# cselab/odil

Measured on AMD Instinct MI355X. Metric: grid-point-updates/s, Poisson 512^3 multigrid, higher is better.
Workload: dtype f64

## Files before the change

### include/odil_hip.h

```cpp
#ifndef ODIL_HIP_H
#define ODIL_HIP_H

#include <stddef.h>
#include <stdint.h>

#ifdef __cplusplus
extern "C" {
#endif

#define ODIL_MAX_NDIM 4
#define ODIL_MAX_LEVELS 32
#define ODIL_E_INVAL (-1)
#define ODIL_E_LAUNCH (-2)
#define ODIL_E_NODEV (-3)

const char* odil_last_error(void);
int odil_version(void);
int odil_device_count(void);
size_t odil_reduce_workspace_bytes(void);

int odil_interp_add_f64(const double* coarse, const double* add, double* fine, const int64_t* cshape, int ndim,
                        const char* loc, double coarse_scale, double add_scale, void* stream);
int odil_interp_add_f32(const float* coarse, const float* add, float* fine, const int64_t* cshape, int ndim,
                        const char* loc, float coarse_scale, float add_scale, void* stream);
// ... 116 lines not shown
size_t odil_poisson_residual_synth_workspace_bytes(const int64_t* cshape);
int odil_poisson_residual_synth_f64(const double* coarse, const double* w0, const double* rhs, double* fu,
                                    const int64_t* cshape, const double* h2, int64_t z0, int64_t z1, double denom,
                                    double* partials, double* column_sums, size_t column_sums_size, double* loss,
                                    void* stream);
int odil_poisson_residual_synth_f32(const float* coarse, const float* w0, const float* rhs, float* fu,
                                    const int64_t* cshape, const float* h2, int64_t z0, int64_t z1, double denom,
                                    double* partials, double* column_sums, size_t column_sums_size, float* loss,
                                    void* stream);

int odil_poisson_jacobi_synth_f64(const double* coarse, const double* x, const double* rhs, double* xout,
                                  const int64_t* cshape, const double* h2, double omega, void* stream);
int odil_poisson_jacobi_synth_f32(const float* coarse, const float* x, const float* rhs, float* xout,
                                  const int64_t* cshape, const float* h2, float omega, void* stream);

int odil_poisson_adjoint_f64(const double* fu, double* gu, const int64_t* shape, int ndim, const double* h2,
                             double scale, void* stream);
int odil_poisson_adjoint_f32(const float* fu, float* gu, const int64_t* shape, int ndim, const float* h2,
                             float scale, void* stream);
int odil_poisson_adjoint_adam_f64(const double* fu, double* gu, double* x, double* m, double* v, const int64_t* shape,
                                  int ndim, const double* h2, double scale, double alpha, double one_minus_b1,
                                  double one_minus_b2, double eps, const double* alpha_dev, void* stream);
int odil_poisson_adjoint_adam_f32(const float* fu, float* gu, float* x, float* m, float* v, const int64_t* shape,
                                  int ndim, const float* h2, float scale, float alpha, float one_minus_b1,
                                  float one_minus_b2, float eps, const float* alpha_dev, void* stream);
int odil_poisson_jac_coeffs_f64(double* coeffs, const int64_t* shape, int ndim, const double* h2, void* stream);
int odil_poisson_jac_coeffs_f32(float* coeffs, const int64_t* shape, int ndim, const float* h2, void* stream);
int odil_poisson_jac_match_f64(const double* const* arrays, const int64_t* shape, int ndim, const double* h2,
                               double* partials, double* out, void* stream);
int odil_poisson_jac_match_f32(const float* const* arrays, const int64_t* shape, int ndim, const float* h2, double* partials,
                               float* out, void* stream);

int odil_adam_step_f64(double* x, double* m, double* v, const double* g, int64_t n, double alpha,
                       double one_minus_b1, double one_minus_b2, double eps, const double* alpha_dev, void* stream);
int odil_adam_step_f32(float* x, float* m, float* v, const float* g, int64_t n, float alpha, float one_minus_b1,
                       float one_minus_b2, float eps, const float* alpha_dev, void* stream);
int odil_adam_step_pieces_f64(double* x, double* m, double* v, const double* g, int64_t npieces, int64_t stride,
                              int64_t offset, int64_t count, double alpha, double one_minus_b1, double one_minus_b2,
                              double eps, const double* alpha_dev, void* stream);
int odil_adam_step_pieces_f32(float* x, float* m, float* v, const float* g, int64_t npieces, int64_t stride,
                              int64_t offset, int64_t count, float alpha, float one_minus_b1, float one_minus_b2,
                              float eps, const float* alpha_dev, void* stream);
int odil_planes_copy_f64(double* arr, double* buf, const int64_t* descs, int ndesc, int64_t max_count, int vec_ok,
                         int mode, void* stream);
int odil_planes_copy_f32(float* arr, float* buf, const int64_t* descs, int ndesc, int64_t max_count, int vec_ok,
                         int mode, void* stream);
int odil_axpy_f64(double* y, const double* x, int64_t n, double a, void* stream);
int odil_axpy_f32(float* y, const float* x, int64_t n, float a, void* stream);
int odil_scale_f64(const double* x, double* y, int64_t n, double a, const double* adev, void* stream);
int odil_scale_f32(const float* x, float* y, int64_t n, float a, const float* adev, void* stream);
int odil_addcmul_f64(double* y, const double* a, const double* b, int64_t n, int accumulate, void* stream);
int odil_addcmul_f32(float* y, const float* a, const float* b, int64_t n, int accumulate, void* stream);
size_t odil_dots_workspace_bytes(int nvec);
int odil_dots_f64(const double* a, int64_t lda, int nvec, const double* b, int64_t n, double* partials,
                  double* out, void* stream);
int odil_dots_f32(const float* a, int64_t lda, int nvec, const float* b, int64_t n, double* partials, float* out,
                  void* stream);
int odil_dots3_f64(const double* a, int64_t lda, int nvec, const double* b0, const double* b1, const double* b2,
                   int64_t n, double* partials, double* out, void* stream);
int odil_dots3_f32(const float* a, int64_t lda, int nvec, const float* b0, const float* b1, const float* b2, int64_t n,
                   double* partials, float* out, void* stream);
int odil_lbfgs_probe_f64(const double* g, const double* d, int64_t n, double* partials, double* out, void* stream);
int odil_lbfgs_probe_f32(const float* g, const float* d, int64_t n, double* partials, float* out, void* stream);
int odil_lincomb_f64(double* y, double beta, const double* a, int64_t lda, int nvec, const double* coef, int64_t n,
                     void* stream);
int odil_lincomb_f32(float* y, float beta, const float* a, int64_t lda, int nvec, const float* coef, int64_t n,
                     void* stream);

int odil_stencil_apply_f64(const double* coeffs, const int64_t* shifts, int nshift, const double* x, double* y,
                           const int64_t* shape, int ndim, int transpose, void* stream);
int odil_stencil_apply_f32(const float* coeffs, const int64_t* shifts, int nshift, const float* x, float* y,
                           const int64_t* shape, int ndim, int transpose, void* stream);
int odil_stencil_march_f64(const double* coeffs, const int64_t* shifts, int nshift, int diag, const double* b, double* x,
                           const int64_t* shape, int ndim, int axis, int direction, void* stream);
int odil_stencil_march_f32(const float* coeffs, const int64_t* shifts, int nshift, int diag, const float* b, float* x,
                           const int64_t* shape, int ndim, int axis, int direction, void* stream);
int odil_stencil_var_smooth_f64(const double* coeffs, const double* x, const double* b, double* out, const int64_t* shape,
                                int ndim, double omega, int mode, void* stream);
int odil_stencil_var_smooth_f32(const float* coeffs, const float* x, const float* b, float* out, const int64_t* shape,
                                int ndim, float omega, int mode, void* stream);
int odil_stencil_var_residual_restrict_f64(const double* coeffs, const double* x, const double* b, double* coarse,
                                           const int64_t* shape, int ndim, double scale, double* partials, double* loss,
                                           void* stream);
int odil_stencil_var_residual_restrict_f32(const float* coeffs, const float* x, const float* b, float* coarse,
                                           const int64_t* shape, int ndim, float scale, double* partials, float* loss,
                                           void* stream);
int odil_stencil_var_residual_restrict_slab_f64(const double* coeffs, const double* x, const double* b, double* coarse,
                                                const int64_t* shape, int ndim, double scale, int64_t z0, int64_t z1,
                                                double denom, double* partials, double* loss, void* stream);
int odil_stencil_var_residual_restrict_slab_f32(const float* coeffs, const float* x, const float* b, float* coarse,
                                                const int64_t* shape, int ndim, float scale, int64_t z0, int64_t z1,
                                                double denom, double* partials, float* loss, void* stream);
int odil_stencil_var_coarsen_f64(const double* coeffs, double* coarse, const int64_t* shape, int ndim, void* stream);
int odil_stencil_var_coarsen_f32(const float* coeffs, float* coarse, const int64_t* shape, int ndim, void* stream);
int odil_stencil_var_coarsen_axes_f64(const double* coeffs, double* coarse, const int64_t* shape, int ndim, const int* halve,
                                      void* stream);
int odil_stencil_var_coarsen_axes_f32(const float* coeffs, float* coarse, const int64_t* shape, int ndim, const int* halve,
                                      void* stream);

int odil_poisson_small_epochs_resident(const int64_t* shapes, int nlvl, int ndim, int elem_size);
int odil_poisson_small_epochs_f64(double* x, double* m, double* v, double* g, double* u, double* fu, const double* rhs,
                                  const int64_t* shapes, int nlvl, int ndim, const double* h2, const double* alphas,
                                  int nepochs, double one_minus_b1, double one_minus_b2, double eps, double* losses,
                                  double* norms, double* partials, void* stream);
int odil_poisson_small_epochs_f32(float* x, float* m, float* v, float* g, float* u, float* fu, const float* rhs,
                                  const int64_t* shapes, int nlvl, int ndim, const float* h2, const float* alphas,
                                  int nepochs, float one_minus_b1, float one_minus_b2, float eps, float* losses,
                                  float* norms, double* partials, void* stream);

int64_t odil_poisson_small_epochs_partials(const int64_t* shapes, int ndim, int elem_size);
int odil_poisson_small_epochs_batch_f64(double* x, double* m, double* v, double* g, double* u, double* fu, const double* rhs,
                                        int nbatch, int64_t state_stride, int64_t field_stride, const int64_t* shapes,
                                        int nlvl, int ndim, const double* h2, const double* alphas, int64_t alpha_stride,
                                        int nepochs, double one_minus_b1, double one_minus_b2, double eps, double* losses,
                                        double* norms, int64_t out_stride, double* partials, int64_t partials_stride,
                                        void* stream);
int odil_poisson_small_epochs_batch_f32(float* x, float* m, float* v, float* g, float* u, float* fu, const float* rhs,
                                        int nbatch, int64_t state_stride, int64_t field_stride, const int64_t* shapes,
                                        int nlvl, int ndim, const float* h2, const float* alphas, int64_t alpha_stride,
                                        int nepochs, float one_minus_b1, float one_minus_b2, float eps, float* losses,
                                        float* norms, int64_t out_stride, double* partials, int64_t partials_stride,
                                        void* stream);

int odil_mg_batch_levels_ok(const int64_t* shapes, int nlvl, int ndim, int nbatch);
int64_t odil_poisson_batch_partials(const int64_t* shape, int ndim, int elem_size);
int odil_poisson_residual_batch_f64(const double* u, const double* rhs, double* fu, int nbatch, int64_t u_stride,
                                    int64_t rhs_stride, int64_t fu_stride, const int64_t* shape, int ndim,
                                    const double* h2, double* partials, int64_t partials_stride, int64_t partials_len,
                                    double* loss, void* stream);
int odil_poisson_residual_batch_f32(const float* u, const float* rhs, float* fu, int nbatch, int64_t u_stride,
                                    int64_t rhs_stride, int64_t fu_stride, const int64_t* shape, int ndim, const float* h2,
                                    double* partials, int64_t partials_stride, int64_t partials_len, float* loss,
                                    void* stream);
int odil_poisson_adjoint_adam_batch_f64(const double* fu, double* gu, double* x, double* m, double* v, int nbatch,
                                        int64_t fu_stride, int64_t g_stride, int64_t x_stride, int64_t m_stride,
                                        int64_t v_stride, const int64_t* shape, int ndim, const double* h2, double scale,
                                        double one_minus_b1, double one_minus_b2, double eps, const double* alpha_dev,
                                        int64_t alpha_stride, void* stream);
int odil_poisson_adjoint_adam_batch_f32(const float* fu, float* gu, float* x, float* m, float* v, int nbatch,
                                        int64_t fu_stride, int64_t g_stride, int64_t x_stride, int64_t m_stride,
                                        int64_t v_stride, const int64_t* shape, int ndim, const float* h2, float scale,
                                        float one_minus_b1, float one_minus_b2, float eps, const float* alpha_dev,
                                        int64_t alpha_stride, void* stream);
int odil_mg_synth_adj_adam_batch_f64(const double* gu, double* const* grads, const int64_t* shapes, int nlvl, int ndim,
                                     int nbatch, double* const* x, double* const* m, double* const* v, double one_minus_b1,
                                     double one_minus_b2, double eps, const double* alpha_dev, int64_t alpha_stride,
                                     void* stream);
int odil_mg_synth_adj_adam_batch_f32(const float* gu, float* const* grads, const int64_t* shapes, int nlvl, int ndim,
                                     int nbatch, float* const* x, float* const* m, float* const* v, float one_minus_b1,
                                     float one_minus_b2, float eps, const float* alpha_dev, int64_t alpha_stride,
                                     void* stream);

int odil_interp_adj_kind(const int64_t* cshape, int ndim, const char* loc, int elem_size);
int odil_mg_volumes_levels_ok(const int64_t* shapes, int nlvl, int ndim, int nbatch, int elem_size);
size_t odil_poisson_residual_synth_batch_workspace_bytes(const int64_t* cshape);
int64_t odil_poisson_residual_synth_batch_partials(const int64_t* cshape);
int odil_poisson_residual_synth_batch_f64(const double* coarse, const double* w0, const double* rhs, double* fu,
                                          int nbatch, int64_t w0_stride, int64_t rhs_stride, int64_t fu_stride,
                                          const int64_t* cshape, int ndim, const double* h2, double* partials,
                                          int64_t partials_stride, int64_t partials_len, double* column_sums,
                                          size_t column_sums_size, double* loss, void* stream);
int odil_poisson_residual_synth_batch_f32(const float* coarse, const float* w0, const float* rhs, float* fu, int nbatch,
                                          int64_t w0_stride, int64_t rhs_stride, int64_t fu_stride,
                                          const int64_t* cshape, int ndim, const float* h2, double* partials,
                                          int64_t partials_stride, int64_t partials_len, double* column_sums,
                                          size_t column_sums_size, float* loss, void* stream);
int odil_poisson_adjoint_adam_volumes_f64(const double* fu, double* gu, double* x, double* m, double* v, int nbatch,
                                          int64_t fu_stride, int64_t g_stride, int64_t x_stride, int64_t m_stride,
                                          int64_t v_stride, const int64_t* shape, int ndim, const double* h2,
                                          double scale, double one_minus_b1, double one_minus_b2, double eps,
                                          const double* alpha_dev, int64_t alpha_stride, void* stream);
int odil_poisson_adjoint_adam_volumes_f32(const float* fu, float* gu, float* x, float* m, float* v, int nbatch,
                                          int64_t fu_stride, int64_t g_stride, int64_t x_stride, int64_t m_stride,
                                          int64_t v_stride, const int64_t* shape, int ndim, const float* h2, float scale,
                                          float one_minus_b1, float one_minus_b2, float eps, const float* alpha_dev,
                                          int64_t alpha_stride, void* stream);
int odil_mg_synth_adj_adam_volumes_f64(const double* gu, double* const* grads, const int64_t* shapes, int nlvl, int ndim,
                                       int nbatch, double* const* x, double* const* m, double* const* v,
                                       double one_minus_b1, double one_minus_b2, double eps, const double* alpha_dev,
                                       int64_t alpha_stride, void* stream);
int odil_mg_synth_adj_adam_volumes_f32(const float* gu, float* const* grads, const int64_t* shapes, int nlvl, int ndim,
                                       int nbatch, float* const* x, float* const* m, float* const* v, float one_minus_b1,
                                       float one_minus_b2, float eps, const float* alpha_dev, int64_t alpha_stride,
                                       void* stream);

int odil_stencil_var_smooth2_f64(const double* coeffs, const double* x, const double* b, double* out, const int64_t* shape,
                                 int ndim, double omega1, double omega2, int zc_hint, void* stream);
int odil_stencil_var_smooth2_f32(const float* coeffs, const float* x, const float* b, float* out, const int64_t* shape,
                                 int ndim, float omega1, float omega2, int zc_hint, void* stream);

int odil_stencil_vcycle_tail_f64(const double* coeffs, const int64_t* shapes, const int* halve, int nlev, int ndim,
                                 const double* xin, const double* b, double* xout, double* work, int64_t work_len,
                                 const double* inv, int ninv, const double* wpre, int npre, const double* wpost,
                                 int npost, int fmg, void* stream);
int odil_stencil_vcycle_tail_f32(const float* coeffs, const int64_t* shapes, const int* halve, int nlev, int ndim,
                                 const float* xin, const float* b, float* xout, float* work, int64_t work_len,
                                 const float* inv, int ninv, const float* wpre, int npre, const float* wpost, int npost,
                                 int fmg, void* stream);
int odil_narrow_scale(const double* x, float* y, int64_t n, double a, const double* msq, void* stream);
int odil_widen_axpy(double* y, const float* x, int64_t n, double a, const double* msq, void* stream);
int odil_max_abs_rows_f64(const double* a, int nrows, int64_t n, double* partials, double* out, void* stream);
int odil_max_abs_rows_f32(const float* a, int nrows, int64_t n, double* partials, float* out, void* stream);
int odil_max_abs_diff_f64(const double* a, const double* b, int64_t n, double* partials, double* out, void* stream);
int odil_max_abs_diff_f32(const float* a, const float* b, int64_t n, double* partials, float* out, void* stream);
int odil_csr_assemble_f64(const double* coeffs, const int64_t* shifts, int nshift, const int64_t* shape, int ndim,
                          int64_t col_offset, int64_t* indptr, int64_t* indices, double* data, void* stream);
int odil_csr_assemble_f32(const float* coeffs, const int64_t* shifts, int nshift, const int64_t* shape, int ndim,
                          int64_t col_offset, int64_t* indptr, int64_t* indices, float* data, void* stream);

size_t odil_dense_block_workspace_bytes(void);
int odil_dense_block_xty_f64(const double* x, const double* y, int64_t n, int px, int py, int64_t ldx, int64_t ldy,
                             double* out, double* workspace, void* stream);
int odil_dense_block_xty_f32(const float* x, const float* y, int64_t n, int px, int py, int64_t ldx, int64_t ldy,
                             float* out, float* workspace, void* stream);
size_t odil_dense_block_wide_workspace_bytes(int px, int py);
int odil_dense_block_xty_wide_f64(const double* x, const double* y, int64_t n, int px, int py, int64_t ldx,
                                  int64_t ldy, double* out, double* workspace, size_t workspace_bytes, void* stream);
int odil_dense_block_xty_wide_f32(const float* x, const float* y, int64_t n, int px, int py, int64_t ldx, int64_t ldy,
                                  float* out, float* workspace, size_t workspace_bytes, void* stream);
int odil_dense_block_gram_f64(const double* d, int64_t n, int p, int64_t ld, double* out, double* workspace,
                              void* stream);
int odil_dense_block_gram_f32(const float* d, int64_t n, int p, int64_t ld, float* out, float* workspace,
                              void* stream);

int odil_bmg_apply_f64(const double* coef, const int64_t* table, const int64_t* desc, const double* x, const double* b,
                       const double* dinv, double* y, int mode, double omega, void* stream);
int odil_bmg_apply_f32(const float* coef, const int64_t* table, const int64_t* desc, const float* x, const float* b,
                       const float* dinv, float* y, int mode, float omega, void* stream);
int odil_bmg_assemble_f64(const double* c1, const double* c2, const int64_t* rmap, const int64_t* ashape,
                          const int64_t* rshape, double* out, void* stream);
int odil_bmg_assemble_f32(const float* c1, const float* c2, const int64_t* rmap, const int64_t* ashape,
                          const int64_t* rshape, float* out, void* stream);
int odil_bmg_transfer_f64(const int64_t* fdesc, const int64_t* cdesc, const int* code, const double* in,
                          const double* add, double* out, int mode, void* stream);
int odil_bmg_transfer_f32(const int64_t* fdesc, const int64_t* cdesc, const int* code, const float* in,
                          const float* add, float* out, int mode, void* stream);
int odil_bmg_galerkin_f64(const int64_t* fdesc, const int64_t* cdesc, const int* code, const double* fcoef,
                          const int64_t* ftable, const int64_t* ctable, int nce, int64_t total, double* ccoef,
                          void* stream);
int odil_bmg_galerkin_f32(const int64_t* fdesc, const int64_t* cdesc, const int* code, const float* fcoef,
                          const int64_t* ftable, const int64_t* ctable, int nce, int64_t total, float* ccoef,
                          void* stream);
int odil_bmg_coarse_dense_f64(const double* coef, const int64_t* table, const int64_t* desc, int64_t np, int64_t lda,
                              double* out, void* stream);
int odil_bmg_coarse_chol_f64(double* work, int64_t n, int64_t np, double tol_rel, double* thr, int* drops,
                             double* inv, void* stream);

#ifdef __cplusplus
}
#endif
#endif
```

### odil_amd/_lib.py

```python

import ctypes
import os
from ctypes import c_char_p, c_double, c_float, c_int, c_int64, c_size_t, c_void_p

import numpy as np
import torch

_HERE = os.path.dirname(os.path.abspath(__file__))
LIB_PATH = os.environ.get("ODIL_HIP_LIB") or os.path.join(_HERE, "libodil_hip.so")

_P = c_void_p
_I64P = ctypes.POINTER(c_int64)

_R = "real"
_SIGNATURES = {
    "interp_add": [_P, _P, _P, _I64P, c_int, c_char_p, _R, _R, _P],
    "interp_adj": [_P, _P, _P, _I64P, c_int, c_char_p, _R, _P],
    "interp_add_ld": [_P, c_int64, _P, _P, _I64P, c_int, c_char_p, _R, _R, _P],
    "interp_adj_ld": [_P, _P, c_int64, _I64P, c_int, c_char_p, _P],
    "interp_adj_cut": [_P, _P, _P, _I64P, c_int, c_char_p, _R, c_int, c_int, _P],
    "interp_adj_cut_adam": [_P, _P, _I64P, c_int, c_char_p, c_int, c_int, _P, _P, _P, _R, _R, _R, _R, _P, _P],
    "restrict": [_P, _P, _I64P, c_int, c_char_p, _P],
    "restrict_adj": [_P, _P, _I64P, c_int, c_char_p, _P],
    "conv_valid": [_P, _P, _P, _I64P, _I64P, _I64P, _I64P, c_int, c_int, _P],
    "mg_synth": [_P, _P, _P, _P, _I64P, c_int, c_int, c_char_p, _P],
    "mg_synth_adj": [_P, _P, _P, _P, _I64P, c_int, c_int, c_char_p, _P],
    "mg_synth_adj_adam": [_P, _P, _P, _P, _I64P, c_int, c_int, c_char_p, _P, _P, _P, _R, _R, _R, _R, _P, _P],
    "field_gather": [_P, _P, _I64P, c_int, c_char_p, c_char_p, _I64P, _P],
    "field_scatter": [_P, _P, _I64P, c_int, c_char_p, c_char_p, _I64P, c_int, _P],
    "mean_reduce": [_P, c_int64, c_int, _P, _P, _P],
    "poisson_residual": [_P, _P, _P, _I64P, c_int, _P, _P, _P, _P],
    "poisson_small_epochs": [_P, _P, _P, _P, _P, _P, _P, _I64P, c_int, c_int, _P, _P, c_int, _R, _R, _R, _P, _P, _P, _P],
    "poisson_small_epochs_batch": [_P, _P, _P, _P, _P, _P, _P, c_int, c_int64, c_int64, _I64P, c_int, c_int, _P, _P, c_int64,
                                   c_int, _R, _R, _R, _P, _P, c_int64, _P, c_int64, _P],
    "poisson_residual_batch": [_P, _P, _P, c_int, c_int64, c_int64, c_int64, _I64P, c_int, _P, _P, c_int64, c_int64, _P, _P],
    "poisson_adjoint_adam_batch": [_P, _P, _P, _P, _P, c_int, c_int64, c_int64, c_int64, c_int64, c_int64, _I64P, c_int, _P,
                                   _R, _R, _R, _R, _P, c_int64, _P],
    "mg_synth_adj_adam_batch": [_P, _P, _I64P, c_int, c_int, c_int, _P, _P, _P, _R, _R, _R, _P, c_int64, _P],
    "poisson_residual_synth_batch": [_P, _P, _P, _P, c_int, c_int64, c_int64, c_int64, _I64P, c_int, _P, _P, c_int64,
                                     c_int64, _P, c_size_t, _P, _P],
    "poisson_adjoint_adam_volumes": [_P, _P, _P, _P, _P, c_int, c_int64, c_int64, c_int64, c_int64, c_int64, _I64P, c_int,
                                     _P, _R, _R, _R, _R, _P, c_int64, _P],
    "mg_synth_adj_adam_volumes": [_P, _P, _I64P, c_int, c_int, c_int, _P, _P, _P, _R, _R, _R, _P, c_int64, _P],
    "poisson_jacobi": [_P, _P, _P, _I64P, c_int, _P, _R, _P],
    "poisson_jacobi2": [_P, _P, _P, _I64P, c_int, _P, _R, _R, c_int, _P],
    "poisson_jacobi2_synth": [_P, _P, _P, _P, _I64P, _P, _R, _R, c_int, _P],
    "poisson_residual_restrict": [_P, _P, _P, _I64P, c_int, _P, _R, _P, _P, _P],
    "poisson_residual_restrict_slab": [_P, _P, _P, _I64P, c_int, _P, _R, c_int64, c_int64, c_double, _P, _P, _P],
    "poisson_residual_synth": [_P, _P, _P, _P, _I64P, _P, c_int64, c_int64, c_double, _P, _P, c_size_t, _P, _P],
    "poisson_jacobi_synth": [_P, _P, _P, _P, _I64P, _P, _R, _P],
    "poisson_residual_slab": [_P, _P, _P, _I64P, c_int, _P, c_int64, c_int64, c_double, _P, _P, _P],
    "poisson_adjoint": [_P, _P, _I64P, c_int, _P, _R, _P],
    "poisson_adjoint_adam": [_P, _P, _P, _P, _P, _I64P, c_int, _P, _R, _R, _R, _R, _R, _P, _P],
    "poisson_adjoint_transpose_adam": [_P, _P, _P, _I64P, _P, _R, _P, _P, _P, _P, _P, _P, _R, _R, _R, _R, _P, c_int,
                                       c_int, _P],
    "poisson_jac_coeffs": [_P, _I64P, c_int, _P, _P],
    "poisson_jac_match": [_P, _I64P, c_int, _P, _P, _P, _P],
    "adam_step": [_P, _P, _P, _P, c_int64, _R, _R, _R, _R, _P, _P],
    "adam_step_pieces": [_P, _P, _P, _P, c_int64, c_int64, c_int64, c_int64, _R, _R, _R, _R, _P, _P],
    "planes_copy": [_P, _P, _P, c_int, c_int64, c_int, c_int, _P],
    "axpy": [_P, _P, c_int64, _R, _P],
    "scale": [_P, _P, c_int64, _R, _P, _P],
    "addcmul": [_P, _P, _P, c_int64, c_int, _P],
    "dots": [_P, c_int64, c_int, _P, c_int64, _P, _P, _P],
    "dots3": [_P, c_int64, c_int, _P, _P, _P, c_int64, _P, _P, _P],
    "lbfgs_probe": [_P, _P, c_int64, _P, _P, _P],
    "lincomb": [_P, _R, _P, c_int64, c_int, _P, c_int64, _P],
    "stencil_apply": [_P, _I64P, c_int, _P, _P, _I64P, c_int, c_int, _P],
    "stencil_march": [_P, _I64P, c_int, c_int, _P, _P, _I64P, c_int, c_int, c_int, _P],
    "stencil_var_smooth": [_P, _P, _P, _P, _I64P, c_int, _R, c_int, _P],
    "stencil_var_smooth2": [_P, _P, _P, _P, _I64P, c_int, _R, _R, c_int, _P],
    "stencil_var_residual_restrict": [_P, _P, _P, _P, _I64P, c_int, _R, _P, _P, _P],
    "stencil_var_residual_restrict_slab": [_P, _P, _P, _P, _I64P, c_int, _R, c_int64, c_int64, c_double, _P, _P, _P],
    "stencil_var_coarsen": [_P, _P, _I64P, c_int, _P],
    "stencil_var_coarsen_axes": [_P, _P, _I64P, c_int, _P, _P],
    "stencil_vcycle_tail": [_P, _I64P, _P, c_int, c_int, _P, _P, _P, _P, c_int64, _P, c_int, _P, c_int, _P, c_int, c_int, _P],
    "max_abs_diff": [_P, _P, c_int64, _P, _P, _P],
    "max_abs_rows": [_P, c_int, c_int64, _P, _P, _P],
    "csr_assemble": [_P, _I64P, c_int, _I64P, c_int, c_int64, _P, _P, _P, _P],
    "dense_block_xty": [_P, _P, c_int64, c_int, c_int, c_int64, c_int64, _P, _P, _P],
    "dense_block_xty_wide": [_P, _P, c_int64, c_int, c_int, c_int64, c_int64, _P, _P, c_size_t, _P],
    "dense_block_gram": [_P, c_int64, c_int, c_int64, _P, _P, _P],
    "bmg_apply": [_P, _P, _I64P, _P, _P, _P, _P, c_int, _R, _P],
    "bmg_assemble": [_P, _P, _P, _I64P, _I64P, _P, _P],
    "bmg_transfer": [_I64P, _I64P, _P, _P, _P, _P, c_int, _P],
    "bmg_galerkin": [_I64P, _I64P, _P, _P, _P, _P, c_int, c_int64, _P, _P],
}

_SIGNATURES_F64 = {
    "bmg_coarse_dense": [_P, _P, _I64P, c_int64, c_int64, _P, _P],
    "bmg_coarse_chol": [_P, c_int64, c_int64, c_double, _P, _P, _P, _P],
}

EXPORTED = [
    "odil_last_error", "odil_version", "odil_device_count", "odil_reduce_workspace_bytes", "odil_dots_workspace_bytes",
    "odil_dense_block_workspace_bytes", "odil_dense_block_wide_workspace_bytes", "odil_narrow_scale", "odil_widen_axpy",
    "odil_poisson_small_epochs_resident", "odil_poisson_small_epochs_partials", "odil_poisson_batch_partials",
    "odil_mg_batch_levels_ok", "odil_poisson_residual_synth_workspace_bytes",
    "odil_mg_volumes_levels_ok", "odil_interp_adj_kind", "odil_poisson_residual_synth_batch_workspace_bytes",
    "odil_poisson_residual_synth_batch_partials",
] + [
    "odil_{}_{}".format(name, suffix) for name in _SIGNATURES for suffix in ("f64", "f32")
] + ["odil_{}_f64".format(name) for name in _SIGNATURES_F64]

_lib = None


class OdilHipError(RuntimeError):
    pass


def load():
    global _lib
    if _lib is not None:
        return _lib
    if not os.path.exists(LIB_PATH):
        raise OdilHipError(
            "HIP extension not built: {} is missing. Run `python -c 'import __graft_entry__ as g; g.build()'` "
            "or `make -C odil_amd/csrc`. There is no CPU fallback.".format(LIB_PATH)
        )
    lib = ctypes.CDLL(LIB_PATH)
    lib.odil_last_error.restype = c_char_p
    lib.odil_last_error.argtypes = []
    lib.odil_version.restype = c_int
    lib.odil_device_count.restype = c_int
    lib.odil_reduce_workspace_bytes.restype = c_size_t
    lib.odil_dots_workspace_bytes.restype = c_size_t
    lib.odil_dots_workspace_bytes.argtypes = [c_int]
    lib.odil_dense_block_workspace_bytes.restype = c_size_t
    lib.odil_dense_block_wide_workspace_bytes.restype = c_size_t
    lib.odil_dense_block_wide_workspace_bytes.argtypes = [c_int, c_int]
    lib.odil_poisson_small_epochs_resident.restype = c_int
    lib.odil_poisson_small_epochs_resident.argtypes = [_I64P, c_int, c_int, c_int]
    lib.odil_poisson_small_epochs_partials.restype = c_int64
    lib.odil_poisson_small_epochs_partials.argtypes = [_I64P, c_int, c_int]
    lib.odil_poisson_batch_partials.restype = c_int64
    lib.odil_poisson_batch_partials.argtypes = [_I64P, c_int, c_int]
    lib.odil_mg_batch_levels_ok.restype = c_int
    lib.odil_mg_batch_levels_ok.argtypes = [_I64P, c_int, c_int, c_int]
    lib.odil_poisson_residual_synth_workspace_bytes.restype = c_size_t
    lib.odil_poisson_residual_synth_workspace_bytes.argtypes = [_I64P]
    lib.odil_interp_adj_kind.restype = c_int
    lib.odil_interp_adj_kind.argtypes = [_I64P, c_int, c_char_p, c_int]
    lib.odil_mg_volumes_levels_ok.restype = c_int
    lib.odil_mg_volumes_levels_ok.argtypes = [_I64P, c_int, c_int, c_int, c_int]
    lib.odil_poisson_residual_synth_batch_workspace_bytes.restype = c_size_t
    lib.odil_poisson_residual_synth_batch_workspace_bytes.argtypes = [_I64P]
    lib.odil_poisson_residual_synth_batch_partials.restype = c_int64
    lib.odil_poisson_residual_synth_batch_partials.argtypes = [_I64P]
    for name in ("odil_narrow_scale", "odil_widen_axpy"):
        fn = getattr(lib, name)
        fn.restype = c_int
        fn.argtypes = [_P, _P, c_int64, c_double, _P, _P]
    for name, sig in _SIGNATURES.items():
        for suffix, real in (("f64", c_double), ("f32", c_float)):
            fn = getattr(lib, "odil_{}_{}".format(name, suffix))
            fn.restype = c_int
            fn.argtypes = [real if a is _R else a for a in sig]
    for name, sig in _SIGNATURES_F64.items():
        fn = getattr(lib, "odil_{}_f64".format(name))
        fn.restype = c_int
        fn.argtypes = sig
    _lib = lib
    return lib


def suffix_of(dtype):
    if dtype == torch.float64:
        return "f64"
    if dtype == torch.float32:
        return "f32"
    raise TypeError("unsupported dtype {} (float32 / float64 only)".format(dtype))


def call(name, dtype, *args, unserved_ok=False):
    fn = _entry.get((name, dtype))
    if fn is None:
        fn = _entry[(name, dtype)] = getattr(load(), "odil_{}_{}".format(name, suffix_of(dtype)))
    status = fn(*args)
    if status == 1 and unserved_ok:
        return False
    if status != 0:
        raise OdilHipError("odil_{}: {} (status {})".format(name, load().odil_last_error().decode(), status))
    return True


_entry = dict()


def ptr(t):
    if t is None:
        return None
    if not isinstance(t, torch.Tensor):
        raise TypeError("expected a torch.Tensor, got {}".format(type(t).__name__))
    if not t.is_cuda:
        raise OdilHipError("tensor is on '{}': the HIP kernels need device memory (no CPU fallback)".format(t.device))
    if not t.is_contiguous():
        raise OdilHipError("tensor must be contiguous (C order)")
    return c_void_p(t.data_ptr())


def i64(values):
    values = [int(v) for v in values]
    return (c_int64 * len(values))(*values)


def ptr_array(tensors):
    arr = (c_void_p * len(tensors))()
    for i, t in enumerate(tensors):
        arr[i] = None if t is None else t.data_ptr()
        if t is not None and (not t.is_cuda or not t.is_contiguous()):
            raise OdilHipError("level arrays must be contiguous device tensors")
    return arr


def host_reals(values, dtype):
    np_dtype = np.float64 if dtype == torch.float64 else np.float32
    arr = np.ascontiguousarray(np.asarray(values, dtype=np_dtype))
    return arr, arr.ctypes.data_as(c_void_p)


def stream_ptr():
    return c_void_p(_raw_stream(_current_device()))


_raw_stream = getattr(torch._C, "_cuda_getCurrentRawStream", None)
_current_device = getattr(torch._C, "_cuda_getDevice", None)
if _raw_stream is None or _current_device is None:
    def stream_ptr():
        return c_void_p(torch.cuda.current_stream().cuda_stream)


def reduce_workspace_elems():
    return load().odil_reduce_workspace_bytes() // 8
```

### odil_amd/backend.py

```python

from argparse import Namespace

import numpy as np
import torch

_NP2T = {
    np.dtype("float32"): torch.float32,
    np.dtype("float64"): torch.float64,
    np.dtype("int32"): torch.int32,
    np.dtype("int64"): torch.int64,
    np.dtype("bool"): torch.bool,
}


def torch_dtype(dtype):
    if dtype is None or isinstance(dtype, torch.dtype):
        return dtype
    if dtype is int:
        return torch.int64
    if dtype is float:
        return torch.float64
    if dtype is bool:
        return torch.bool
    return _NP2T[np.dtype(dtype)]


def numpy_dtype(dtype):
    if isinstance(dtype, torch.dtype):
        return {v: k for k, v in _NP2T.items()}[dtype]
    return np.dtype(dtype)


class _ConvValidFn(torch.autograd.Function):

    @staticmethod
    def forward(ctx, x, w, strides, transposed, out_shape):
        from . import ops

        ctx.save_for_backward(w)
        ctx.strides, ctx.transposed, ctx.xshape = strides, transposed, tuple(x.shape)
        return ops.conv_valid(x, w, strides, transposed=transposed, out_shape=out_shape)

    @staticmethod
    def backward(ctx, g):
        (w,) = ctx.saved_tensors
        g = g.contiguous()
        if ctx.transposed:
            gx = _ConvValidFn.apply(g, w, ctx.strides, False, None)
            gx = gx[tuple(slice(0, n) for n in ctx.xshape)]
        else:
            gx = _ConvValidFn.apply(g, w, ctx.strides, True, ctx.xshape)
        return gx, None, None, None, None


class ModRocm:

    def __init__(self, device=None):
        if device is None:
            device = torch.device("cuda", torch.cuda.current_device()) if torch.cuda.is_available() else None
        if device is None:
            raise RuntimeError(
                "odil_amd needs a HIP device (MI355X): none is visible and there is no CPU fallback. "
                "Pass ModRocm(device='cpu') only to exercise host-side plumbing in tests."
            )
        self.device = torch.device(device)
        self.mod = self
        self.jax = None
        self.tf = None
        self.modsp = None
        self.float32 = np.float32
        self.float64 = np.float64
        self.int32 = np.int32
        self.ndarray = torch.Tensor
        self.batch_to_space = None
        self.random = Namespace()
        self._gen = torch.Generator(device="cpu")
        self.random.set_seed = self._set_seed
        self.random.uniform = self._uniform
        self.random.normal = self._normal

    def _t(self, x, dtype=None):
        dtype = torch_dtype(dtype)
        if isinstance(x, torch.Tensor):
            if x.device != self.device:
                x = x.to(self.device)
            return x if dtype is None or x.dtype == dtype else x.to(dtype)
        if isinstance(x, (bool, int, float, np.bool_, np.integer, np.floating)):
            if dtype is None:
                dtype = (torch.bool if isinstance(x, (bool, np.bool_)) else torch.int64 if isinstance(x, (int, np.integer))
                         else torch_dtype(np.asarray(x).dtype))
            return torch.full((), x, dtype=dtype, device=self.device)
        return torch.as_tensor(np.asarray(x), device=self.device).to(dtype) if dtype is not None else torch.as_tensor(
            np.asarray(x), device=self.device
        )

    def cast(self, x, dtype):
        return self._t(x, dtype)

    def array(self, x, dtype=None):
        return self._t(x, dtype)

    constant = array
    native = array

    def variable(self, x, dtype=None):
        return self._t(x, dtype).detach().clone().contiguous()

    def numpy(self, x):
        if isinstance(x, torch.Tensor):
            return x.detach().cpu().numpy()
        return np.asarray(x)

    def spnative(self, x):
        return x

    def is_tensor(self, x):
        return isinstance(x, torch.Tensor)

    def copy(self, x):
        return self._t(x).clone()

    def stop_gradient(self, x):
        return self._t(x).detach()

    @staticmethod
    def _shape(shape):
        if isinstance(shape, (int, np.integer)):
            return (int(shape),)
        return tuple(int(s) for s in shape)

    def zeros(self, shape, dtype=None):
        return torch.zeros(self._shape(shape), dtype=torch_dtype(dtype or np.float32), device=self.device)

    def ones(self, shape, dtype=None):
        return torch.ones(self._shape(shape), dtype=torch_dtype(dtype or np.float32), device=self.device)

    def full(self, shape, value, dtype=None):
        return torch.full(self._shape(shape), value, dtype=torch_dtype(dtype), device=self.device)

    def zeros_like(self, x):
        return torch.zeros_like(self._t(x))

    def ones_like(self, x):
        return torch.ones_like(self._t(x))

    def arange(self, *args, dtype=None):
        return torch.arange(*args, dtype=torch_dtype(dtype), device=self.device)

    def linspace(self, start, stop, num=50, endpoint=True, dtype=None):
        return self._t(np.linspace(start, stop, num, endpoint=endpoint, dtype=dtype))

    def meshgrid(self, *xx, indexing="ij"):
        return [self._t(x) for x in np.meshgrid(*[self.numpy(x) for x in xx], indexing=indexing)]

    def reshape(self, x, shape):
        return self._t(x).reshape(self._shape(shape))

# ... 212 lines not shown
```

### odil_amd/core.py

```python

import math
import os
import pickle

import numpy as np
import torch
from torch.autograd.function import once_differentiable

from . import ops
from .backend import ModRocm, numpy_dtype, torch_dtype


def assert_equal(first, second, msg=""):
    if not (first == second):
        raise ValueError("Expected equal '{:}' and '{:}'{}".format(first, second, msg))


class Field:
    def __init__(self, array=None, loc=None, cshape=None):
        self.array = array
        self.loc = loc
        self.cshape = cshape

    def __repr__(self):
        return "odil.Field({}, loc='{}', cshape={:})".format(repr(self.array), self.loc, self.cshape)

    __str__ = __repr__


class MultigridField:
    def __init__(self, terms=None, loc=None, factors=None, axes=None, method=None):
        self.terms = terms
        self.loc = loc
        self.factors = factors
        self.axes = axes
        self.method = method


class NeuralNet:
    def __init__(self, weights=None, biases=None, func_in=None, func_out=None, activation=None):
        self.weights = weights
        self.biases = biases
        self.func_in = func_in
        self.func_out = func_out
        self.activation = activation or "tanh"


class Array:
    def __init__(self, array=None, shape=None):
        self.array = array
        self.shape = shape

    def __repr__(self):
        return "odil.Array({}, shape={:})".format(repr(self.array), self.shape)

    __str__ = __repr__


class State:
    def __init__(self, fields=None, initialized=False):
        self.fields = fields if fields is not None else dict()
        self.initialized = initialized


class _MgSynthFn(torch.autograd.Function):
    @staticmethod
    def forward(ctx, loc, factors, *terms):
        ctx.loc, ctx.factors = loc, factors
        ctx.shapes = [tuple(t.shape) for t in terms]
        return ops.mg_synth([t.contiguous() for t in terms], loc, factors=factors)

    @staticmethod
    @once_differentiable
    def backward(ctx, gu):
        grads = ops.mg_synth_adj(gu.contiguous(), ctx.shapes, ctx.loc, factors=ctx.factors)
        return (None, None) + tuple(grads)


class _FieldAccessFn(torch.autograd.Function):
    @staticmethod
    def forward(ctx, src, field_loc, shift, loc):
        ctx.meta = (tuple(src.shape), field_loc, shift, loc)
        return ops.field_gather(src.contiguous(), field_loc, shift, loc)

    @staticmethod
    @once_differentiable
    def backward(ctx, g):
        shape, field_loc, shift, loc = ctx.meta
        return ops.field_scatter(g.contiguous(), shape, field_loc, shift, loc), None, None, None


class _MeanFn(torch.autograd.Function):

    @staticmethod
    def forward(ctx, x, square):
        x = x.contiguous()
        ctx.square = square
        ctx.save_for_backward(x)
        return ops.mean_reduce(x, square=square)

    @staticmethod
    @once_differentiable
    def backward(ctx, gout):
        (x,) = ctx.saved_tensors
        n = x.numel()
        gout = gout.contiguous().to(x.dtype)
        if ctx.square:
            return ops.scale(x, 2.0 / n, adev=gout.reshape(1)), None
        return ops.scale(torch.ones_like(x), 1.0 / n, adev=gout.reshape(1)), None


class _InterpFn(torch.autograd.Function):
    @staticmethod
    def forward(ctx, u, loc):
        ctx.loc, ctx.shape = loc, tuple(u.shape)
        return ops.interp_add(u.contiguous(), loc)

    @staticmethod
    @once_differentiable
    def backward(ctx, g):
        return ops.interp_adj(g.contiguous(), ctx.loc, ctx.shape), None


class _RestrictFn(torch.autograd.Function):
    @staticmethod
    def forward(ctx, u, loc):
        ctx.loc, ctx.shape = loc, tuple(u.shape)
        return ops.restrict_to_coarser(u.contiguous(), loc)

    @staticmethod
    @once_differentiable
    def backward(ctx, g):
        return ops.restrict_adj(g.contiguous(), ctx.loc, ctx.shape), None


def _as_tensor(u, mod):
    if isinstance(u, torch.Tensor):
        return u
    mod = mod or _default_mod()
    return mod.array(u)


def _default_mod():
    from . import runtime

    return runtime.get_mod()


def interp_to_finer(u, loc=None, method=None, mod=None, depth=1):
    method = method or "stack"
    if method not in ["conv", "stack"]:
        raise ValueError("Unknown method='{}'".format(method))
    u = _as_tensor(u, mod)
    loc = loc or "c" * u.dim()
    assert_equal(len(loc), u.dim())
    for l in loc:
        assert l in "cn.", "Invalid loc={}".format(loc)
    for _ in range(depth):
        u = _InterpFn.apply(u, loc)
    return u


def restrict_to_coarser(u, loc=None, method=None, mod=None, depth=1):
# ... 587 lines not shown
            off = self.key_to_offset[key]
            if kind == "dense":
                m = modsp.csr_array(payload.cpu().numpy())
                block = modsp.csr_array((m.data, m.indices + off, m.indptr), shape=(nrows, self.ncols))
            else:
                coeff, shift, loc, vshape = payload
                field = self.key_to_field[key]
                size = self.key_to_size[key]
                cols = (torch.arange(size, dtype=torch.float64, device=self.device) + off).reshape(field.array.shape)
                cols = ops.field_gather(cols.contiguous(), field.loc, shift, loc).reshape(-1).cpu().numpy()
                rows = np.arange(nrows)
                block = modsp.csr_array(
                    (coeff.reshape(-1).cpu().numpy(), (rows, cols.astype(np.int64))), shape=(nrows, self.ncols)
                )
            full = modsp.vstack(
                [modsp.csr_array((row0, self.ncols), dtype=npdt), block,
                 modsp.csr_array((self.nrows - row0 - nrows, self.ncols), dtype=npdt)]
            ).tocsr()
            matrix = matrix + full
        return matrix.tocsr()


class Problem:
    def __init__(self, operator, domain, extra=None, tracers=None, jit=None):
        self.domain = domain
        self.operator = operator
        self.extra = extra
        if tracers is None:
            tracers = dict()
        if "epoch" not in tracers:
            tracers["epoch"] = 0
        self.tracers = tracers
        if jit is None:
            from . import runtime

            jit = runtime.enable_jit
        self.jit = jit
        self._names = None
        self._fused = None
        self._fused_checked = False
        self._traced = None
        self._jac_traced = None
        if not isinstance(domain.mod, ModRocm):
            raise NotImplementedError("Unsupported mod={:}".format(domain.mod))

    @staticmethod
    def _split_outputs(ff):
        assert isinstance(ff, (tuple, list)) and len(ff), "Operator must return a non-empty list"
        names = [f[0] if isinstance(f, tuple) else "" for f in ff]
        nonempty = [name for name in names if name]
        assert len(nonempty) == len(set(nonempty)), "Name of fields must be unique, got {}".format(nonempty)
        values = [f[1] if isinstance(f, tuple) else f for f in ff]
        return names, values

    def _shadow_state(self, state, arrays):
        fields = dict()
        for key, field in state.fields.items():
            if isinstance(field, Field):
                fields[key] = Field(None, loc=field.loc, cshape=field.cshape)
            elif isinstance(field, MultigridField):
                fields[key] = MultigridField(
                    [Field(None, loc=t.loc, cshape=t.cshape) for t in field.terms], loc=field.loc,
                    factors=field.factors, axes=field.axes, method=field.method,
                )
            elif isinstance(field, NeuralNet):
                fields[key] = NeuralNet(list(field.weights), list(field.biases), func_in=field.func_in,
                                        func_out=field.func_out, activation=field.activation)
            elif isinstance(field, Array):
                fields[key] = Array(None, field.shape)
            else:
                raise TypeError("Unknown field type '{}'".format(type(field).__name__))
        shadow = State(fields=fields, initialized=True)
        self.domain.arrays_to_state(arrays, shadow)
        return shadow

    def recognise(self, state):
        if not self._fused_checked:
            self._fused_checked = True
            from . import fused, runtime

            if runtime.enable_fuse:
                self._fused = fused.detect(self, state)
            if self._fused is None and runtime.enable_trace:
                from . import stencil_jit

                self._traced = stencil_jit.trace(self, state)

    def eval_loss_grad_device(self, state):
        if not state.initialized:
            raise RuntimeError("Uninitialized state, use `state = domain.init_state(state)`")
        self.recognise(state)
        if self._fused is not None:
            return self._fused.eval_loss_grad(state)
        if self._traced is not None:
            if not self._traced.matches(state):
                from . import stencil_jit

                self._traced = stencil_jit.trace(self, state)
            if self._traced is not None:
                return self._traced.eval_loss_grad(state)
        if self.jit:
            return self._eval_loss_grad_graph(state)
        return self._eval_loss_grad_generic(state)

    def _eval_loss_grad_graph(self, state):
        domain = self.domain
        arrays = domain.arrays_from_state(state)
        key = tuple((tuple(a.shape), a.dtype) for a in arrays)
        cache = self.__dict__.setdefault("_graph_cache", dict())
        entry = cache.get(key)
        if entry is False:
            return self._eval_loss_grad_generic(state)
        if entry is None:
            try:
                entry = self._capture_graph(state, arrays)
            except Exception as e:
                from .util import printlog

                printlog("odil_amd: hipGraph capture failed ({}: {}); using the eager path".format(
                    type(e).__name__, str(e).splitlines()[0] if str(e) else ""))
                torch.cuda.synchronize()
                cache[key] = False
                return self._eval_loss_grad_generic(state)
            cache[key] = entry
        static_in, static_tr, graph, out = entry
        for s_, a in zip(static_in, arrays):
            if s_.data_ptr() != a.data_ptr():
                s_.copy_(a)
        for k, t in static_tr.items():
            t.fill_(self.tracers[k])
        graph.replay()
        loss, grads, terms, names, norms = out
        return loss, list(grads), list(terms), names, list(norms)

    def _capture_graph(self, state, arrays):
        static_in = [a.detach().clone() for a in arrays]
        static_tr = dict()
        live_tracers = dict(self.tracers)
        for k, v in self.tracers.items():
            if isinstance(v, (int, float, np.integer, np.floating)) and not isinstance(v, bool):
                static_tr[k] = torch.tensor(float(v), dtype=torch_dtype(self.domain.dtype), device=self.domain.mod.device)
                live_tracers[k] = static_tr[k]
        static_state = self._shadow_state(state, static_in)
        saved = self.tracers
        try:
            self.tracers = live_tracers
            side = torch.cuda.Stream()
            side.wait_stream(torch.cuda.current_stream())
            with torch.cuda.stream(side):
                for _ in range(2):
                    self._eval_loss_grad_generic(static_state)
            torch.cuda.current_stream().wait_stream(side)
            graph = torch.cuda.CUDAGraph()
            with torch.cuda.graph(graph):
                out = self._eval_loss_grad_generic(static_state)
        finally:
            self.tracers = saved
        return static_in, static_tr, graph, out

    def _eval_loss_grad_generic(self, state):
        domain = self.domain
        arrays = domain.arrays_from_state(state)
        leaves = [a.detach().requires_grad_(True) for a in arrays]
        shadow = self._shadow_state(state, leaves)
        with torch.enable_grad():
            ctx = Context(domain, shadow, extra=self.extra, tracers=self.tracers)
            names, values = self._split_outputs(self.operator(ctx))
            terms = [
                _MeanFn.apply(v.value, False) if isinstance(v, Context.Raw) else _MeanFn.apply(v, True)
                for v in values
            ]
            loss = terms[0]
            for t in terms[1:]:
                loss = loss + t
        grads = torch.autograd.grad(loss, leaves, allow_unused=True)
        grads = [g if g is not None else torch.zeros_like(a) for g, a in zip(grads, arrays)]
        loss = loss.detach()
        terms = [t.detach() for t in terms]
        norms = [t if isinstance(v, Context.Raw) else torch.sqrt(t) for t, v in zip(terms, values)]
        self._names = names
        return loss, grads, terms, names, norms

    def eval_loss_grad(self, state):
        loss, grads, terms, names, norms = self.eval_loss_grad_device(state)
        to_np = lambda t: np.array(t.detach().cpu().numpy()) if isinstance(t, torch.Tensor) else np.array(t)
        return to_np(loss), grads, list(map(to_np, terms)), names, list(map(to_np, norms))

    def eval_operator(self, state):
        if not state.initialized:
            raise RuntimeError("Uninitialized state, use `state = domain.init_state(state)`")
        with torch.no_grad():
            ctx = Context(self.domain, state, extra=self.extra, tracers=self.tracers)
            names, values = self._split_outputs(self.operator(ctx))
            values = [v.value if isinstance(v, Context.Raw) else v for v in values]
        return values, names

    def eval_operator_grad(self, state):
        if not state.initialized:
            raise RuntimeError("Uninitialized state, use `state = domain.init_state(state)`")
        domain = self.domain
        from . import runtime

        if runtime.enable_trace and int(os.environ.get("ODIL_TRACE_JAC", 1)) and torch.cuda.is_available():
            if self._jac_traced is None or (self._jac_traced and not self._jac_traced.matches(state)):
                from . import stencil_jit

                self._jac_traced = stencil_jit.trace_jacobian(self, state) or False
            if self._jac_traced:
                return self._jac_traced.eval_operator_grad(state)
        arrays = domain.arrays_from_state(state)
        leaves = [a.detach().requires_grad_(True) for a in arrays]
        shadow = self._shadow_state(state, leaves)
        with torch.enable_grad():
            ctx = Context(domain, shadow, extra=self.extra, tracers=self.tracers, distinct_shift=True)
            names, values = self._split_outputs(self.operator(ctx))
            values = [v.value if isinstance(v, Context.Raw) else v for v in values]
            grads = []
            for v in values:
                g = dict()
                descs = list(ctx.desc_to_array.keys())
                symbols = [ctx.desc_to_array[d] for d in descs]
                if v.requires_grad and symbols:
                    gg = torch.autograd.grad(v.sum(), symbols, retain_graph=True, allow_unused=True)
                else:
                    gg = [None] * len(symbols)
                g.update(dict(zip(descs, gg)))
                for jkey, arr in ctx.key_to_array_jac.items():
                    g[jkey] = self._dense_jacobian(v, arr)
                grads.append(g)
        values = [v.detach() for v in values]
        return values, grads, names

    @staticmethod
    def _dense_jacobian(v, arr):
        arrs = arr if isinstance(arr, list) else [arr]
        if not v.requires_grad:
            return [None for _ in arrs] if isinstance(arr, list) else None
        flat = v.reshape(-1)
        nparam = sum(int(a.numel()) for a in arrs)
        jacs = None
        if nparam < flat.numel():
            try:
                w = torch.ones_like(v).requires_grad_(True)
                gg = torch.autograd.grad(v, arrs, grad_outputs=w, create_graph=True, allow_unused=True)
                jacs = []
                for g, a in zip(gg, arrs):
                    if g is None:
                        jacs.append(torch.zeros(tuple(v.shape) + tuple(a.shape), dtype=v.dtype, device=v.device))
                        continue
                    if not g.requires_grad:
                        raise RuntimeError("first reverse pass is not differentiable")
                    gflat = g.reshape(-1)
                    cols = [torch.autograd.grad(gflat[e], w, retain_graph=True)[0] for e in range(gflat.numel())]
                    jacs.append(torch.stack(cols, dim=-1).reshape(tuple(v.shape) + tuple(a.shape)))
            except RuntimeError:
                jacs = None
        if jacs is None:
            rows = [[] for _ in arrs]
            for i in range(flat.numel()):
                gg = torch.autograd.grad(flat[i], arrs, retain_graph=True, allow_unused=True)
                for k, (g, a) in enumerate(zip(gg, arrs)):
                    rows[k].append(g if g is not None else torch.zeros_like(a))
            jacs = [torch.stack(r).reshape(tuple(v.shape) + tuple(a.shape)) for r, a in zip(rows, arrs)]
        if all(float(j.abs().max()) == 0 for j in jacs):
            return [None for _ in arrs] if isinstance(arr, list) else None
        return jacs if isinstance(arr, list) else jacs[0]

    def linearize_device(self, state):
        if not state.initialized:
            raise RuntimeError("Uninitialized state, use `state = domain.init_state(state)`")
        values, grads, names = self.eval_operator_grad(state)
        op = LinearizedOperator(self.domain, state)
        for value, grad in zip(values, grads):
            op.add_output(tuple(value.shape), grad)
        vector = values[0].reshape(-1) if len(values) == 1 else torch.cat([v.reshape(-1) for v in values])
        return vector, op

    def linearize(self, state, modsp=None):
        vector, op = self.linearize_device(state)
        return vector, op.to_scipy(modsp)

    def get_context(self, state):
        return self.domain.get_context(state, extra=self.extra, tracers=self.tracers)


def _to_numpy(a):
    return a.detach().cpu().numpy() if isinstance(a, torch.Tensor) else np.array(a)


def checkpoint_save(domain, state, path):
    fields = dict()
    for key in state.fields:
        fields[key] = [_to_numpy(a) for a in domain.arrays_from_field(state.fields[key])]
    with open(path, "wb") as f:
        pickle.dump({"fields": fields}, f)


def checkpoint_load(domain, state, path, skip_missing=True, keys=None):
    with open(path, "rb") as f:
        stored = pickle.load(f).get("fields", dict())
    wanted = list(state.fields) if not keys else list(keys)
    missing = [key for key in wanted if key not in stored]
    if missing and not skip_missing:
        raise RuntimeError(f"Field {missing[0]} not found in {path}")
    for key in wanted:
        if key in stored:
            entry = stored[key]
# ... 26 lines not shown
```

### odil_amd/csrc/common.h

```cpp
#pragma once

#include <hip/hip_runtime.h>
#include <stdint.h>
#include <stdio.h>
#include <string.h>

#include "odil_hip.h"

namespace odil {

constexpr int kNumXcd = 8;
constexpr int kBlock = 256;
constexpr int kMaxPartials = 65536;
constexpr int kDotPartials = 1024;
constexpr int64_t kStreamBytes = (int64_t)128 << 20;
constexpr int kGridCap = 2048;

void set_error(const char* fmt, ...);

inline int check_launch(const char* what) {
  hipError_t err = hipGetLastError();
  if (err != hipSuccess) {
    set_error("%s: %s", what, hipGetErrorString(err));
    return ODIL_E_LAUNCH;
  }
  return 0;
}

enum Loc : int { kNone = 0, kCell = 1, kNode = 2 };

inline int parse_loc(const char* loc, int ndim, int out[4]) {
  if (!loc || (int)strlen(loc) != ndim) return ODIL_E_INVAL;
  for (int i = 0; i < 4; ++i) out[i] = kNone;
  for (int i = 0; i < ndim; ++i) {
    char c = loc[i];
    int v = c == 'c' ? kCell : c == 'n' ? kNode : c == '.' ? kNone : -1;
    if (v < 0) return ODIL_E_INVAL;
    out[4 - ndim + i] = v;
  }
  return 0;
}

inline void canon_shape(const int64_t* shape, int ndim, int64_t out[4]) {
  for (int i = 0; i < 4; ++i) out[i] = 1;
  for (int i = 0; i < ndim; ++i) out[4 - ndim + i] = shape[i];
}

inline int64_t prod4(const int64_t n[4]) { return n[0] * n[1] * n[2] * n[3]; }

inline int flat_grid_cap() { return 1 << 20; }

inline int grid_flat(int64_t work_items, int per_block) {
  int64_t nb = (work_items + per_block - 1) / per_block;
  if (nb > flat_grid_cap()) nb = flat_grid_cap();
  if (nb < 1) nb = 1;
  return (int)nb;
}

inline int grid_for(int64_t work_items, int per_block) {
  int64_t nb = (work_items + per_block - 1) / per_block;
  if (nb > kGridCap) nb = kGridCap;
  if (nb < 1) nb = 1;
  return (int)nb;
}

struct RowSched {
  int Z, Y, XS;
  int Yc;
};

inline RowSched make_sched(int64_t Z, int64_t Y, int64_t XS) {
  RowSched s;
  s.Z = (int)Z;
  s.Y = (int)Y;
  s.XS = (int)XS;
  s.Yc = (int)((Y + kNumXcd - 1) / kNumXcd);
  return s;
}

inline bool sched_ok(int64_t Z, int64_t Y, int64_t XS) { return Z * Y * XS < (int64_t)1 << 31; }

inline int sched_grid(const RowSched& s) {
  int64_t per_xcd = (int64_t)s.Z * s.Yc * s.XS;
  int64_t cap = kGridCap / kNumXcd;
  if (per_xcd > cap) per_xcd = cap;
  if (per_xcd < 1) per_xcd = 1;
  return (int)(per_xcd * kNumXcd);
}

struct UnitSched {
  int ZCH, Y, XS;
  int ZC;
  int axis;
  int chunk;
  int per_xcd;
};

inline UnitSched make_unit_sched_chunked(int64_t Z, int64_t Y, int64_t XS, int zc) {
  UnitSched s;
  s.ZC = zc;
  s.ZCH = (int)((Z + zc - 1) / zc);
  s.Y = (int)Y;
  s.XS = (int)XS;
  if (Y >= 4 * kNumXcd) {
    s.axis = 1;
    s.chunk = (int)((Y + kNumXcd - 1) / kNumXcd);
    s.per_xcd = s.ZCH * s.chunk * s.XS;
  } else if (s.ZCH >= kNumXcd) {
    s.axis = 0;
    s.chunk = 0;
    s.per_xcd = (int)(((int64_t)s.ZCH * s.Y * s.XS + kNumXcd - 1) / kNumXcd);
  } else {
    s.axis = -1;
    s.chunk = 0;
    s.per_xcd = s.ZCH * s.Y * s.XS;
  }
  return s;
}

inline UnitSched make_unit_sched(int64_t Z, int64_t Y, int64_t XS, int64_t target_units = 2 * kGridCap) {
  int64_t zc = (Z * Y * XS) / target_units;
  if (zc < 1) zc = 1;
  if (zc > 64) zc = 64;
  if (zc > Z) zc = Z;
  return make_unit_sched_chunked(Z, Y, XS, (int)zc);
}

inline int unit_grid(const UnitSched& s) { return s.axis < 0 ? s.per_xcd : s.per_xcd * kNumXcd; }

#ifdef __HIPCC__
__device__ inline bool unit_decode(const UnitSched& s, int& zc, int& y, int& xs) {
  if (s.axis < 0) {
    const int i = blockIdx.x;
    xs = i % s.XS;
    const int r = i / s.XS;
    y = r % s.Y;
    zc = r / s.Y;
    return true;
  }
  const int k = blockIdx.x % kNumXcd, i = blockIdx.x / kNumXcd;
  xs = i % s.XS;
  const int r = i / s.XS;
  if (s.axis == 1) {
    y = k * s.chunk + r % s.chunk;
    zc = r / s.chunk;
    return y < s.Y;
  }
  const int u = k * s.per_xcd + i;
  xs = u % s.XS;
  const int ru = u / s.XS;
  y = ru % s.Y;
  zc = ru / s.Y;
  return zc < s.ZCH;
}
#endif

#ifdef __HIPCC__
struct RowIter {
  int t, step, count, y0, ny;
};

__device__ inline RowIter sched_begin(const RowSched& s) {
  RowIter it;
  const int k = blockIdx.x % kNumXcd;
  it.t = blockIdx.x / kNumXcd;
  it.step = gridDim.x / kNumXcd;
  it.y0 = k * s.Yc;
  int y1 = it.y0 + s.Yc;
  if (y1 > s.Y) y1 = s.Y;
  it.ny = y1 > it.y0 ? y1 - it.y0 : 0;
  it.count = s.Z * it.ny * s.XS;
  return it;
}

template <typename I>
__device__ inline void sched_decode(const RowSched& s, const RowIter& it, I& z, I& y, I& xs) {
  const int per_plane = it.ny * s.XS;
  const int zi = it.t / per_plane;
  const int r = it.t - zi * per_plane;
  const int yl = r / s.XS;
  z = zi;
  xs = r - yl * s.XS;
  y = it.y0 + yl;
}

__device__ inline double block_sum(double v) {
  __shared__ double wave_sums[kBlock / 64];
  for (int off = 32; off > 0; off >>= 1) v += __shfl_down(v, off, 64);
  int lane = threadIdx.x & 63, wave = threadIdx.x >> 6;
  __syncthreads();
  if (lane == 0) wave_sums[wave] = v;
  __syncthreads();
  double total = 0;
  if (threadIdx.x == 0) {
    for (int w = 0; w < kBlock / 64; ++w) total += wave_sums[w];
  }
  return total;
}
#endif

#ifdef __HIPCC__
__device__ inline int lane_shift_word(int v, bool up) {
  return up ? __builtin_amdgcn_update_dpp(0, v, 0x138, 0xf, 0xf, false)
            : __builtin_amdgcn_update_dpp(0, v, 0x130, 0xf, 0xf, false);
}
__device__ inline float from_prev_lane(float v) { return __int_as_float(lane_shift_word(__float_as_int(v), true)); }
__device__ inline float from_next_lane(float v) { return __int_as_float(lane_shift_word(__float_as_int(v), false)); }
__device__ inline double from_prev_lane(double v) {
  const int lo = lane_shift_word(__double2loint(v), true), hi = lane_shift_word(__double2hiint(v), true);
  return __hiloint2double(hi, lo);
}
__device__ inline double from_next_lane(double v) {
  const int lo = lane_shift_word(__double2loint(v), false), hi = lane_shift_word(__double2hiint(v), false);
  return __hiloint2double(hi, lo);
}
#endif

template <typename T>
struct AdamArgs {
  T* x;
  T* m;
  T* v;
  T alpha, omb1, omb2, eps;
  const T* alpha_dev;
  int64_t alpha_stride;
  int member_axis;
};

#ifdef __HIPCC__
template <typename T>
__device__ inline void adam_update(T& x, T& m, T& v, T g, const AdamArgs<T>& a, int64_t member = 0) {
  m = m + (g - m) * a.omb1;
  v = v + (g * g - v) * a.omb2;
  const T alpha = a.alpha_dev ? a.alpha_dev[member * a.alpha_stride] : a.alpha;
  x = x - (m * alpha) / (sqrt(v) + a.eps);
}
#endif

template <typename T>
int adam_launch(T* x, T* m, T* v, const T* g, int64_t n, T alpha, T omb1, T omb2, T eps, hipStream_t stream,
                const T* alpha_dev = nullptr);

template <typename T>
int launch_final_reduce(const double* partials, int count, int stride, int nq, double scale, T* out,
                        hipStream_t stream);

}
```

### odil_amd/csrc/mg_march.hip

```cpp
#include "mg_march.h"
#include "poisson.h"

namespace odil {

template <typename T, int CX>
__device__ inline void acc_plane(T (&s)[2][2 * CX], const T (&v)[3][CX + 2], int wz) {
#pragma unroll
  for (int sy = 0; sy < 2; ++sy)
#pragma unroll
    for (int sx = 0; sx < 2 * CX; ++sx) {
      T t = s[sy][sx];
#pragma unroll
      for (int ry = 0; ry < 2; ++ry)
#pragma unroll
        for (int rx = 0; rx < 2; ++rx) {
          const int w = wz * (sy == ry ? 1 : 3) * ((sx & 1) == rx ? 1 : 3);
          t = t + T(w) * v[sy + ry][(sx >> 1) + (sx & 1) + rx];
        }
      s[sy][sx] = t;
    }
}

template <typename T, int CX>
__device__ inline void zero_plane(T (&s)[2][2 * CX]) {
// ... 473 lines not shown
      T c1[1][CX], r1[1][CX];
      reduce_planes<T, CX, 6, 1>(gfine, f1, fnz, fplane, fny, fnx, jy, jx0, ay, ax, c1, r1);
#pragma unroll
      for (int c = 0; c < CX; ++c) {
        rc[p][c] = c1[0][c];
        rr[p][c] = r1[0][c];
      }
    }
  } else {
    reduce_planes<T, CX, 4, NP>(gfine, f, fnz, fplane, fny, fnx, jy, jx0, ay, ax, rc, rr);
  }
}

template <typename T, int CX>
__device__ inline void reduce_pair(const T* __restrict__ gfine, const int (&f)[2], int fnz, int64_t fplane, int fny,
                                   int fnx, int jy, int jx0, const Adj6& ay, const Adj6 (&ax)[CX], T (&rc)[2][CX],
                                   T (&rr)[2][CX]) {
  if constexpr (CX == 1) {
    reduce_dispatch<T, CX, 2>(gfine, f, fnz, fplane, fny, fnx, jy, jx0, ay, ax, rc, rr);
  } else {
#pragma unroll
    for (int p = 0; p < 2; ++p) {
      const int f1[1] = {f[p]};
      T c1[1][CX], r1[1][CX];
      reduce_dispatch<T, CX, 1>(gfine, f1, fnz, fplane, fny, fnx, jy, jx0, ay, ax, c1, r1);
#pragma unroll
      for (int c = 0; c < CX; ++c) {
        rc[p][c] = c1[0][c];
        rr[p][c] = r1[0][c];
      }
    }
  }
}

template <typename T>
__device__ inline T combine_z(const T (&wc)[6], const T (&wr)[6], int jz, int cnz, int fnz, bool xy_special,
                              int cut_lo, int cut_hi) {
  const bool z_special = ((jz == 0 || jz == 1) && !cut_lo) || ((jz == cnz - 2 || jz == cnz - 1) && !cut_hi);
  if (!z_special && !xy_special) return (T(0.25) * wc[1] + T(0.75) * wc[2]) + (T(0.75) * wc[3] + T(0.25) * wc[4]);
  if (!z_special) {
    T sc = T(0), sr = T(0);
    const T zw[6] = {T(0), T(0.25), T(0.75), T(0.75), T(0.25), T(0)};
#pragma unroll
    for (int i = 0; i < 6; ++i) {
      sc = sc + zw[i] * wc[i];
      sr = sr + zw[i] * wr[i];
    }
    return T(2) * sc - sr;
  }
  T sc = T(0), sr = T(0);
#pragma unroll
  for (int i = 0; i < 6; ++i) {
    const int k = 2 * jz - 2 + i;
    const float w = w_cell(jz, k, fnz), lo = w_cell(-1, k, fnz), hi = w_cell(cnz, k, fnz);
    const float zc_w = w + (jz == 0 && !cut_lo ? lo : 0.f) + (jz == cnz - 1 && !cut_hi ? hi : 0.f);
    const float zr_w = w + (jz == 1 && !cut_lo ? lo : 0.f) + (jz == cnz - 2 && !cut_hi ? hi : 0.f);
    sc = sc + T(zc_w) * wc[i];
    sr = sr + T(zr_w) * wr[i];
  }
  return T(2) * sc - sr;
}

template <typename T>
__device__ inline void emit_coarse(T* __restrict__ gcoarse, T* __restrict__ gscaled, int64_t ci, T v, T scale,
                                   const AdamArgs<T>& ad) {
  gcoarse[ci] = v;
  if (gscaled) gscaled[ci] = scale * v;
  if (ad.x) {
    T xv = ad.x[ci], mv = ad.m[ci], vv = ad.v[ci];
    adam_update<T>(xv, mv, vv, gscaled ? scale * v : v, ad);
    ad.x[ci] = xv;
    ad.m[ci] = mv;
    ad.v[ci] = vv;
  }
}

template <typename T, int CX>
__device__ inline void put2(T (&wc)[CX][6], T (&wr)[CX][6], int at, const T (&c2)[2][CX], const T (&r2)[2][CX]) {
#pragma unroll
  for (int c = 0; c < CX; ++c) {
    wc[c][at] = c2[0][c], wc[c][at + 1] = c2[1][c];
    wr[c][at] = r2[0][c], wr[c][at + 1] = r2[1][c];
  }
}

template <typename T, int CX>
__device__ inline void slide(T (&wc)[CX][6], T (&wr)[CX][6]) {
#pragma unroll
  for (int c = 0; c < CX; ++c)
#pragma unroll
    for (int i = 0; i < 4; ++i) {
      wc[c][i] = wc[c][i + 2];
      wr[c][i] = wr[c][i + 2];
    }
}

template <int CX>
__device__ inline void column_taps(int jx0, int cnx, Adj6 (&ax)[CX]) {
#pragma unroll
  for (int c = 0; c < CX; ++c) ax[c] = adj6(jx0 + c, cnx);
}

template <typename T, int CX>
__global__ __launch_bounds__(kBlock) void k_interp_adj_march(const T* __restrict__ gfine, T* __restrict__ gcoarse,
                                                             T* __restrict__ gscaled, MarchArgs a, T scale,
                                                             AdamArgs<T> ad) {
  const int cnz = a.cn[0], cny = a.cn[1], cnx = a.cn[2];
  const int fnz = a.fn[0], fny = a.fn[1], fnx = a.fn[2];
  const int64_t cplane = (int64_t)cny * cnx, fplane = (int64_t)fny * fnx;
  int z0, z1, jy, jx0;
  if (!march_decode<CX>(a, z0, z1, jy, jx0)) return;
  Adj6 ax[CX];
  column_taps<CX>(jx0, cnx, ax);
  const Adj6 ay = adj6(jy, cny);
  T wc[CX][6], wr[CX][6];
  {
    T c2[2][CX], r2[2][CX];
    const int fa[2] = {2 * z0 - 2, 2 * z0 - 1}, fb[2] = {2 * z0, 2 * z0 + 1};
    reduce_pair<T, CX>(gfine, fa, fnz, fplane, fny, fnx, jy, jx0, ay, ax, c2, r2);
    put2<T, CX>(wc, wr, 0, c2, r2);
    reduce_pair<T, CX>(gfine, fb, fnz, fplane, fny, fnx, jy, jx0, ay, ax, c2, r2);
    put2<T, CX>(wc, wr, 2, c2, r2);
  }
  for (int jz = z0; jz < z1; ++jz) {
    {
      T c2[2][CX], r2[2][CX];
      const int fn2[2] = {2 * jz + 2, 2 * jz + 3};
      reduce_pair<T, CX>(gfine, fn2, fnz, fplane, fny, fnx, jy, jx0, ay, ax, c2, r2);
      put2<T, CX>(wc, wr, 4, c2, r2);
    }
    const int64_t ci = (int64_t)jz * cplane + (int64_t)jy * cnx + jx0;
#pragma unroll
    for (int c = 0; c < CX; ++c) {
      const T v = combine_z<T>(wc[c], wr[c], jz, cnz, fnz, ax[c].special || ay.special, a.cut_lo, a.cut_hi);
      emit_coarse<T>(gcoarse, gscaled, ci + c, v, scale, ad);
    }
    slide<T, CX>(wc, wr);
  }
}

#ifndef ODIL_ADJ_UNITS
#define ODIL_ADJ_UNITS kGridCap
#endif
#ifndef ODIL_ADJ_UNITS_SMALL
#define ODIL_ADJ_UNITS_SMALL (kGridCap / 4)
#endif
#ifndef ODIL_TILE_Y
#define ODIL_TILE_Y 8
#define ODIL_TILE_X 32
#endif
#ifndef ODIL_TILE_UNITS
#define ODIL_TILE_UNITS (kGridCap / 2)
#endif
constexpr int kTileY = ODIL_TILE_Y, kTileX = ODIL_TILE_X;
constexpr int kTileR = 2 * kTileY + 4, kTileC = 2 * kTileX + 4;
constexpr int kTilePacks = kTileR * (kTileC / 2);
constexpr int kTileLoads = (kTilePacks + kBlock - 1) / kBlock;
static_assert(kTileY * kTileX == kBlock, "one thread per coarse column of the tile");
constexpr int kTileRS = kTileC / 2 + 2;
constexpr int kTileLds = kTileR * kTileRS + 64;
constexpr bool kTileStrips = (kBlock / 64) * (64 / kTileY) == kTileX;
__device__ __forceinline__ void tile_column(int& lx, int& ly) {
  if constexpr (kTileStrips) {
    constexpr int W = 64 / kTileY;
    const int wave = threadIdx.x >> 6, lane = threadIdx.x & 63;
    lx = wave * W + lane % W;
    ly = lane / W;
  } else {
    lx = threadIdx.x % kTileX;
    ly = threadIdx.x / kTileX;
  }
}

template <typename T, int CX = 1>
struct TileVec {
  typedef T type __attribute__((ext_vector_type(2 * CX)));
};

template <typename T, int CX = 1>
__device__ __forceinline__ void tile_fetch(const T* __restrict__ gfine, int fz0, int fnz, int64_t fplane,
                                           const int64_t (&src)[kTileLoads],
                                           typename TileVec<T, CX>::type (&pre)[2][kTileLoads]) {
#pragma unroll
  for (int q = 0; q < 2; ++q) {
    int fz = fz0 + q;
    fz = fz < 0 ? 0 : (fz >= fnz ? fnz - 1 : fz);
    const T* gp = gfine + (int64_t)fz * fplane;
#pragma unroll
    for (int i = 0; i < kTileLoads; ++i)
      pre[q][i] = *reinterpret_cast<const typename TileVec<T, CX>::type*>(gp + src[i]);
  }
}

template <typename T>
struct TileCtx {
  const T* gfine;
  T* gcoarse;
  T* gscaled;
  int cnz, cny, cnx, fnz, z0, jy, jx, lx, ly;
  bool sx, sy;
  int cut_lo, cut_hi;
  int64_t cplane, fplane;
  bool owner;
  T scale;
};

template <int CX>
__device__ __forceinline__ void tile_tables_store(float* __restrict__ wt, const Adj6& ay, const Adj6 (&ax)[CX]) {
#pragma unroll
  for (int i = 0; i < 6; ++i) {
    wt[i * kBlock + threadIdx.x] = ay.wc[i];
    wt[(6 + i) * kBlock + threadIdx.x] = ay.wr[i];
#pragma unroll
    for (int cc = 0; cc < CX; ++cc) {
      wt[(12 + 12 * cc + i) * kBlock + threadIdx.x] = ax[cc].wc[i];
      wt[(18 + 12 * cc + i) * kBlock + threadIdx.x] = ax[cc].wr[i];
    }
  }
}
template <int CX>
__device__ __forceinline__ void tile_tables_load(const float* __restrict__ wt, Adj6& ay, Adj6 (&ax)[CX]) {
#pragma unroll
  for (int i = 0; i < 6; ++i) {
    ay.wc[i] = wt[i * kBlock + threadIdx.x];
    ay.wr[i] = wt[(6 + i) * kBlock + threadIdx.x];
#pragma unroll
    for (int cc = 0; cc < CX; ++cc) {
      ax[cc].wc[i] = wt[(12 + 12 * cc + i) * kBlock + threadIdx.x];
      ax[cc].wr[i] = wt[(18 + 12 * cc + i) * kBlock + threadIdx.x];
    }
  }
}

template <typename T, int CX = 1, int RS = kTileRS>
__device__ __forceinline__ void tile_reduce_emit(const TileCtx<T>& c,
                                                 const typename TileVec<T, CX>::type* __restrict__ tile0,
                                                 const typename TileVec<T, CX>::type* __restrict__ tile1, int k,
                                                 bool live, T (&wc)[CX][6], T (&wr)[CX][6], const AdamArgs<T>& ad,
                                                 const float* __restrict__ wt = nullptr,
                                                 const T* __restrict__ cpre = nullptr, int lxl = -1) {
  typedef typename TileVec<T, CX>::type P2;
  constexpr int NV = 2 * CX;
  if (lxl < 0) lxl = c.lx;
  const int f2[2] = {2 * (c.z0 - 1 + k), 2 * (c.z0 - 1 + k) + 1};
  T c2[2][CX], r2[2][CX];
  const bool xy_special = c.sx || c.sy;
  const bool wave_sy = __any(c.sy);
  if (xy_special && !wave_sy) {
    Adj6 ax[CX];
    if (wt) {
#pragma unroll
      for (int i = 0; i < 6; ++i)
#pragma unroll
        for (int cc = 0; cc < CX; ++cc) {
          ax[cc].wc[i] = wt[(12 + 12 * cc + i) * kBlock + threadIdx.x];
          ax[cc].wr[i] = wt[(18 + 12 * cc + i) * kBlock + threadIdx.x];
        }
    } else {
      column_taps<CX>(c.jx, c.cnx, ax);
    }
#pragma unroll
    for (int q = 0; q < 2; ++q) {
      const P2* tq = q == 0 ? tile0 : tile1;
      const bool inside = f2[q] >= 0 && f2[q] < c.fnz;
      T sc[CX], sr[CX];
#pragma unroll
      for (int cc = 0; cc < CX; ++cc) sc[cc] = sr[cc] = T(0);
#pragma unroll
      for (int r = 0; r < 4; ++r) {
        const P2* row = tq + (2 * c.ly + 1 + r) * RS + lxl;
        const P2 g[3] = {row[0], row[1], row[2]};
#pragma unroll
        for (int cc = 0; cc < CX; ++cc) {
          T xc = T(0), xr = T(0);
#pragma unroll
          for (int i = 0; i < 6; ++i) {
            const int e = NV - 2 + 2 * cc + i;
            const T val = g[e / NV][e % NV];
            xc = xc + T(ax[cc].wc[i]) * val;
            xr = xr + T(ax[cc].wr[i]) * val;
          }
          const T wy = T((r == 0 || r == 3) ? 0.25 : 0.75);
          sc[cc] = sc[cc] + wy * xc;
          sr[cc] = sr[cc] + wy * xr;
        }
      }
#pragma unroll
      for (int cc = 0; cc < CX; ++cc) c2[q][cc] = inside ? sc[cc] : T(0), r2[q][cc] = inside ? sr[cc] : T(0);
    }
  } else if (xy_special) {
    Adj6 ax[CX], ay;
    if (wt) {
      tile_tables_load<CX>(wt, ay, ax);
      ay.special = c.sy;
#pragma unroll
      for (int cc = 0; cc < CX; ++cc) ax[cc].special = c.jx + cc < 2 || c.jx + cc >= c.cnx - 2;
    } else {
      column_taps<CX>(c.jx, c.cnx, ax);
      ay = adj6(c.jy, c.cny);
    }
#pragma unroll
    for (int q = 0; q < 2; ++q) {
      const P2* tq = q == 0 ? tile0 : tile1;
      const int f1[1] = {f2[q]};
      T c1[1][CX], r1[1][CX];
      PackN<T, NV> g[1][6][3];
#pragma unroll
      for (int r = 0; r < 6; ++r)
#pragma unroll
        for (int w = 0; w < 3; ++w) {
          const P2 t = tq[(2 * c.ly + r) * RS + lxl + w];
#pragma unroll
          for (int e = 0; e < NV; ++e) g[0][r][w].e[e] = t[e];
        }
      reduce_loaded<T, CX, 6, 1>(g, f1, c.fnz, ay, ax, c1, r1);
#pragma unroll
      for (int cc = 0; cc < CX; ++cc) c2[q][cc] = c1[0][cc], r2[q][cc] = r1[0][cc];
    }
  } else {
#pragma unroll
    for (int q = 0; q < 2; ++q) {
      const P2* tq = q == 0 ? tile0 : tile1;
      const bool inside = f2[q] >= 0 && f2[q] < c.fnz;
      T sc[CX];
#pragma unroll
      for (int cc = 0; cc < CX; ++cc) sc[cc] = T(0);
#pragma unroll
      for (int r = 0; r < 4; ++r) {
        const T* rowv = reinterpret_cast<const T*>(tq + (2 * c.ly + 1 + r) * RS + lxl);
        const P2 own = *reinterpret_cast<const P2*>(rowv + NV);
        T val[NV + 2];
        val[0] = rowv[NV - 1];
#pragma unroll
        for (int e = 0; e < NV; ++e) val[1 + e] = own[e];
        val[NV + 1] = rowv[2 * NV];
#pragma unroll
        for (int cc = 0; cc < CX; ++cc) {
          T xc = T(0);
          xc = xc + T(0.25) * val[2 * cc];
          xc = xc + T(0.75) * val[2 * cc + 1];
          xc = xc + T(0.75) * val[2 * cc + 2];
          xc = xc + T(0.25) * val[2 * cc + 3];
          sc[cc] = sc[cc] + T((r == 0 || r == 3) ? 0.25 : 0.75) * xc;
        }
      }
#pragma unroll
      for (int cc = 0; cc < CX; ++cc) c2[q][cc] = r2[q][cc] = inside ? sc[cc] : T(0);
    }
  }
  put2<T, CX>(wc, wr, 4, c2, r2);
  if (k >= 2 && c.owner && live) {
    const int jz = c.z0 + k - 2;
    const int64_t ci = (int64_t)jz * c.cplane + (int64_t)c.jy * c.cnx + c.jx;
#pragma unroll
    for (int cc = 0; cc < CX; ++cc) {
      const T v = combine_z<T>(wc[cc], wr[cc], jz, c.cnz, c.fnz, xy_special, c.cut_lo, c.cut_hi);
      if (cpre && ad.x) {
        c.gcoarse[ci + cc] = v;
        T xe = cpre[3 * cc], me = cpre[3 * cc + 1], ve = cpre[3 * cc + 2];
        adam_update<T>(xe, me, ve, v, ad);
        ad.x[ci + cc] = xe, ad.m[ci + cc] = me, ad.v[ci + cc] = ve;
      } else {
        emit_coarse<T>(c.gcoarse, c.gscaled, ci + cc, v, c.scale, ad);
      }
    }
  }
  slide<T, CX>(wc, wr);
}

template <typename T, int CX = 1>
__device__ __forceinline__ void tile_stage(const TileCtx<T>& c, typename TileVec<T, CX>::type* __restrict__ tile0,
                                           typename TileVec<T, CX>::type* __restrict__ tile1, int k, int ahead,
                                           bool live, const int64_t (&src)[kTileLoads], const int (&dst)[kTileLoads],
                                           typename TileVec<T, CX>::type (&pre)[2][kTileLoads], T (&wc)[CX][6],
                                           T (&wr)[CX][6], const AdamArgs<T>& ad, const float* __restrict__ wt) {
  __syncthreads();
#pragma unroll
  for (int i = 0; i < kTileLoads; ++i) {
    tile0[dst[i]] = pre[0][i];
    tile1[dst[i]] = pre[1][i];
  }
  __syncthreads();
  tile_fetch<T, CX>(c.gfine, 2 * (c.z0 - 1 + k + ahead), c.fnz, c.fplane, src, pre);
  tile_reduce_emit<T, CX>(c, tile0, tile1, k, live, wc, wr, ad, wt);
}

template <typename T, int CX>
__global__ __launch_bounds__(kBlock) void k_interp_adj_tile(const T* __restrict__ gfine, T* __restrict__ gcoarse,
                                                            T* __restrict__ gscaled, MarchArgs a, T scale,
                                                            AdamArgs<T> ad) {
  typedef typename TileVec<T, CX>::type P2;
  constexpr int NV = 2 * CX;
  __shared__ P2 tile[2][kTileLds];
  __shared__ float wtab[12 * (CX + 1) * kBlock];
  const int cny = a.cn[1], fny = a.fn[1], fnx = a.fn[2];
  int zc, yt, xt;
  if (!unit_decode(a.usched, zc, yt, xt)) return;
  TileCtx<T> c;
  c.cnz = a.cn[0], c.cnx = a.cn[2], c.fnz = a.fn[0];
  c.cut_lo = a.cut_lo, c.cut_hi = a.cut_hi;
  c.cplane = (int64_t)cny * c.cnx, c.fplane = (int64_t)fny * fnx;
  const int64_t cvol = (int64_t)blockIdx.y * c.cnz * c.cplane, fvol = (int64_t)blockIdx.y * c.fnz * c.fplane;
  gfine += fvol;
  c.gfine = gfine, c.gcoarse = gcoarse + cvol, c.gscaled = gscaled ? gscaled + cvol : nullptr;
  if (ad.x) ad.x += cvol, ad.m += cvol, ad.v += cvol;
  if (ad.alpha_dev) ad.alpha_dev += (int64_t)blockIdx.y * ad.alpha_stride;
  c.scale = scale;
  c.z0 = zc * a.usched.ZC;
  const int z1 = c.z0 + a.usched.ZC < c.cnz ? c.z0 + a.usched.ZC : c.cnz;
  tile_column(c.lx, c.ly);
  c.jy = yt * kTileY + c.ly, c.jx = (xt * kTileX + c.lx) * CX;
  c.owner = c.jy < cny && c.jx < c.cnx;
  c.cny = cny;
  c.sx = c.owner && (c.jx < 2 || c.jx + CX - 1 >= c.cnx - 2);
  c.sy = c.owner && (c.jy < 2 || c.jy >= cny - 2);
  if (c.sx || c.sy) {
    Adj6 ax[CX];
    column_taps<CX>(c.jx, c.cnx, ax);
    tile_tables_store<CX>(wtab, adj6(c.jy, cny), ax);
  }
  int64_t src[kTileLoads];
  int dst[kTileLoads];
#pragma unroll
  for (int k = 0; k < kTileLoads; ++k) {
    const int p = threadIdx.x + k * kBlock;
    const int r = p < kTilePacks ? p / (kTileC / 2) : 0, cc = p < kTilePacks ? p - r * (kTileC / 2) : 0;
    dst[k] = p < kTilePacks ? r * kTileRS + cc : kTileR * kTileRS + (threadIdx.x & 63);
    int fy = 2 * yt * kTileY - 2 + r, fx = NV * (xt * kTileX - 1 + cc);
    fy = fy < 0 ? 0 : (fy >= fny ? fny - 1 : fy);
    fx = fx < 0 ? 0 : (fx >= fnx ? fnx - NV : fx);
    src[k] = (int64_t)fy * fnx + fx;
  }
  T wc[CX][6], wr[CX][6];
#pragma unroll
  for (int cc = 0; cc < CX; ++cc)
#pragma unroll
    for (int i = 0; i < 6; ++i) wc[cc][i] = wr[cc][i] = T(0);
  const int npairs = z1 - c.z0 + 2;
  P2 pre[2][kTileLoads];
  tile_fetch<T, CX>(gfine, 2 * (c.z0 - 1), c.fnz, c.fplane, src, pre);
  for (int k = 0; k < npairs; ++k) {
    tile_stage<T, CX>(c, tile[0], tile[1], k, 1, true, src, dst, pre, wc, wr, ad, wtab);
  }
}

constexpr int kFuR = 2 * kTileY + 6;
constexpr int kFuC = kTileX + 4;
constexpr int kFuPacks = kFuR * kFuC;
constexpr int kFuLoads = (kFuPacks + kBlock - 1) / kBlock;
constexpr int kGC = kTileC / 2;
constexpr int kG0Steps = (kTileR * kFuC + kBlock - 1) / kBlock;
constexpr int kOwnLoads = 2 * kTileY * kTileX / kBlock;

template <typename T>
__device__ __forceinline__ void fu_fetch(const T* __restrict__ fu, int fz0, int fnz, int64_t fplane,
                                         const int64_t (&src)[kFuLoads], typename TileVec<T>::type (&pre)[2][kFuLoads]) {
#pragma unroll
  for (int q = 0; q < 2; ++q) {
    int fz = fz0 + q;
    fz = fz < 0 ? 0 : (fz >= fnz ? fnz - 1 : fz);
    const T* gp = fu + (int64_t)fz * fplane;
#pragma unroll
    for (int i = 0; i < kFuLoads; ++i) pre[q][i] = *reinterpret_cast<const typename TileVec<T>::type*>(gp + src[i]);
  }
}

template <typename T>
__device__ __forceinline__ void fu_publish(typename TileVec<T>::type* __restrict__ ring, int fz0,
                                           const typename TileVec<T>::type (&pre)[2][kFuLoads], T scale) {
#pragma unroll
  for (int q = 0; q < 2; ++q) {
    typename TileVec<T>::type* slot = ring + ((fz0 + q + 8) & 3) * kFuPacks;
#pragma unroll
    for (int i = 0; i < kFuLoads; ++i) {
      const int p = threadIdx.x + i * kBlock;
      if (p < kFuPacks) slot[p] = scale * pre[q][i];
    }
  }
}

template <typename T, bool MUL>
__device__ __forceinline__ T lap_inner(T fb, T fm, T fp, const H2<T>& h, int ax) {
  const T s = (fp + fm) + T(-2) * fb;
  if constexpr (MUL) return s * h.inv[ax];
  return div_h2<T>(s, h, ax);
}

template <typename T, bool MUL, bool G0>
__global__ __launch_bounds__(kBlock) void k_poisson_adjoint_tile(const T* __restrict__ fu, T* __restrict__ g0out_,
                                                                 T* __restrict__ gcoarse, MarchArgs a, H2<T> h,
                                                                 T scale, AdamArgs<T> ad0, T* __restrict__ x1,
                                                                 T* __restrict__ m1, T* __restrict__ v1) {
  T* const g0out = G0 ? g0out_ : nullptr;
  AdamArgs<T> ad1 = ad0;
  ad1.x = x1, ad1.m = m1, ad1.v = v1;
  typedef typename TileVec<T>::type P2;
  __shared__ P2 ring[4 * kFuPacks];
  __shared__ P2 gt[2][kTileR * kTileRS];
  const int cny = a.cn[1], fny = a.fn[1], fnx = a.fn[2];
  int zc, yt, xt;
  if (!unit_decode(a.usched, zc, yt, xt)) return;
  if constexpr (MUL) h.mul_ok[0] = h.mul_ok[1] = h.mul_ok[2] = 1;
  if (ad0.alpha_dev) ad0.alpha = *ad0.alpha_dev;
  ad0.alpha_dev = nullptr;
  ad1.alpha = ad0.alpha, ad1.alpha_dev = nullptr;
  TileCtx<T> c;
  c.gfine = nullptr, c.gcoarse = gcoarse, c.gscaled = nullptr;
  c.cnz = a.cn[0], c.cnx = a.cn[2], c.fnz = a.fn[0];
  c.cut_lo = a.cut_lo, c.cut_hi = a.cut_hi;
  c.cplane = (int64_t)cny * c.cnx, c.fplane = (int64_t)fny * fnx;
  c.scale = T(1);
  c.z0 = zc * a.usched.ZC;
  const int z1 = c.z0 + a.usched.ZC < c.cnz ? c.z0 + a.usched.ZC : c.cnz;
  tile_column(c.lx, c.ly);
  c.jy = yt * kTileY + c.ly, c.jx = xt * kTileX + c.lx;
  c.owner = c.jy < cny && c.jx < c.cnx;
  c.cny = cny;
  c.sx = c.owner && (c.jx < 2 || c.jx >= c.cnx - 2);
  c.sy = c.owner && (c.jy < 2 || c.jy >= cny - 2);
  const int fy0 = 2 * yt * kTileY, fx0 = 2 * xt * kTileX;
  const bool tile_inner = fy0 >= 4 && fy0 + 2 * kTileY + 4 <= fny && fx0 >= 4 && fx0 + 2 * kTileX + 4 <= fnx;
  int64_t src[kFuLoads];
#pragma unroll
  for (int i = 0; i < kFuLoads; ++i) {
    int p = threadIdx.x + i * kBlock;
    p = p < kFuPacks ? p : kFuPacks - 1;
    const int r = p / kFuC, cc = p - r * kFuC;
    int fy = fy0 - 3 + r, fx = fx0 - 4 + 2 * cc;
    fy = fy < 0 ? 0 : (fy >= fny ? fny - 1 : fy);
    fx = fx < 0 ? 0 : (fx >= fnx ? fnx - 2 : fx);
    src[i] = (int64_t)fy * fnx + fx;
  }
  T wc[1][6], wr[1][6];
#pragma unroll
  for (int i = 0; i < 6; ++i) wc[0][i] = wr[0][i] = T(0);
  const int npairs = z1 - c.z0 + 2;
  P2 pre[2][kFuLoads];
  fu_fetch<T>(fu, 2 * (c.z0 - 1) - 1, c.fnz, c.fplane, src, pre);
  fu_publish<T>(ring, 2 * (c.z0 - 1) - 1, pre, scale);
  fu_fetch<T>(fu, 2 * (c.z0 - 1) + 1, c.fnz, c.fplane, src, pre);
  int64_t own_off[kOwnLoads];
#pragma unroll
  for (int i = 0; i < kOwnLoads; ++i) {
    const int o = threadIdx.x + i * kBlock;
    const int row = o / kTileX, cc = o - row * kTileX;
    const int y = fy0 + row, x = fx0 + 2 * cc;
    own_off[i] = y < fny && x < fnx ? (int64_t)y * fnx + x : -1;
  }
  P2 xv[kOwnLoads], mv[kOwnLoads], vv[kOwnLoads];
#pragma unroll
  for (int i = 0; i < kOwnLoads; ++i) xv[i] = mv[i] = vv[i] = P2{T(0), T(0)};
  bool pending = false;
  for (int k = 0; k < npairs; ++k) {
    const int m = c.z0 - 1 + k, zA = 2 * m;
    fu_publish<T>(ring, zA + 1, pre, scale);
    __syncthreads();
    fu_fetch<T>(fu, zA + 3, c.fnz, c.fplane, src, pre);
    T cpre[3] = {T(0), T(0), T(0)};
    if (k >= 2 && c.owner && ad1.x) {
      const int64_t ci = (int64_t)(c.z0 + k - 2) * c.cplane + (int64_t)c.jy * c.cnx + c.jx;
      cpre[0] = ad1.x[ci], cpre[1] = ad1.m[ci], cpre[2] = ad1.v[ci];
    }
#pragma unroll 1
    for (int q = 0; q < 2; ++q) {
      const int z = zA + q;
      if (pending) {
        const P2* gprev = gt[q ^ 1];
        const int64_t zoff = (int64_t)(z - 1) * c.fplane;
#pragma unroll
        for (int i = 0; i < kOwnLoads; ++i) {
          const int o = threadIdx.x + i * kBlock;
          const int row = o / kTileX, cc = o - row * kTileX;
          if (own_off[i] < 0) continue;
          const P2 g = gprev[(row + 2) * kTileRS + cc + 1];
          const int64_t off = zoff + own_off[i];
          if (g0out) __builtin_nontemporal_store(g, reinterpret_cast<P2*>(g0out + off));
          if (ad0.x) {
            P2 xn = xv[i], mn = mv[i], vn = vv[i];
#pragma unroll
            for (int e = 0; e < 2; ++e) {
              T xe = xn[e], me = mn[e], ve = vn[e];
              adam_update<T>(xe, me, ve, g[e], ad0);
              xn[e] = xe, mn[e] = me, vn[e] = ve;
            }
            __builtin_nontemporal_store(xn, reinterpret_cast<P2*>(ad0.x + off));
            __builtin_nontemporal_store(mn, reinterpret_cast<P2*>(ad0.m + off));
            __builtin_nontemporal_store(vn, reinterpret_cast<P2*>(ad0.v + off));
          }
        }
      }
      pending = z >= 2 * c.z0 && z < 2 * z1;
      if (pending && ad0.x) {
        const int64_t zoff = (int64_t)z * c.fplane;
#pragma unroll
        for (int i = 0; i < kOwnLoads; ++i) {
          const int64_t off = zoff + (own_off[i] < 0 ? 0 : own_off[i]);
          xv[i] = __builtin_nontemporal_load(reinterpret_cast<const P2*>(ad0.x + off));
          mv[i] = __builtin_nontemporal_load(reinterpret_cast<const P2*>(ad0.m + off));
          vv[i] = __builtin_nontemporal_load(reinterpret_cast<const P2*>(ad0.v + off));
        }
      }
      const P2* pm = ring + ((z - 1 + 8) & 3) * kFuPacks;
      const P2* pc = ring + ((z + 8) & 3) * kFuPacks;
      const P2* pp = ring + ((z + 1 + 8) & 3) * kFuPacks;
      P2* gq = gt[q];
      const int zj = z + (c.cut_lo ? 2 : 0), zn = c.fnz + (c.cut_lo ? 2 : 0) + (c.cut_hi ? 2 : 0);
      const bool z_in = z >= 0 && z < c.fnz;
      if (tile_inner && z_in && zj >= 2 && zj < zn - 2) {
#pragma unroll 1
        for (int i = 0; i < kG0Steps; ++i) {
          const int w = threadIdx.x + i * kBlock;
          const int r = w / kFuC, cc = w - r * kFuC;
          if (r < kTileR && cc < kGC) {
            const int at = w + kFuC + 1;
            const P2 fc = pc[at], fl = pc[at - 1], fr = pc[at + 1];
            const P2 fym = pc[at - kFuC], fyp = pc[at + kFuC], fzm = pm[at], fzp = pp[at];
            P2 g;
#pragma unroll
            for (int e = 0; e < 2; ++e) {
              const T fb = fc[e];
              T acc = T(0);
              acc = acc + lap_inner<T, MUL>(fb, fzm[e], fzp[e], h, 0);
              acc = acc + lap_inner<T, MUL>(fb, fym[e], fyp[e], h, 1);
              acc = acc + lap_inner<T, MUL>(fb, e == 0 ? fl[1] : fc[0], e == 0 ? fc[1] : fr[0], h, 2);
              g[e] = acc;
            }
            gq[r * kTileRS + cc] = g;
          }
        }
      } else {
#pragma unroll 1
        for (int i = 0; i < kG0Steps; ++i) {
          const int w = threadIdx.x + i * kBlock;
          const int r = w / kFuC, cc = w - r * kFuC;
          if (r < kTileR && cc < kGC) {
            const int y = fy0 - 2 + r, x = fx0 - 2 + 2 * cc;
            const int at = w + kFuC + 1;
            P2 g;
            g[0] = T(0), g[1] = T(0);
            if (z_in && y >= 0 && y < fny && x >= 0 && x < fnx) {
              const P2 fc = pc[at], fl = pc[at - 1], fr = pc[at + 1];
              const P2 fym = pc[at - kFuC], fyp = pc[at + kFuC], fzm = pm[at], fzp = pp[at];
#pragma unroll
              for (int e = 0; e < 2; ++e) {
                const T fb = fc[e];
                T acc = T(0);
                acc = acc + adj_axis<T>(fb, fzm[e], fzp[e], zj, zn, h, 0);
                acc = acc + adj_axis<T>(fb, fym[e], fyp[e], y, fny, h, 1);
                acc = acc + adj_axis<T>(fb, e == 0 ? fl[1] : fc[0], e == 0 ? fc[1] : fr[0], x + e, fnx, h, 2);
                g[e] = acc;
              }
            }
            gq[r * kTileRS + cc] = g;
          }
        }
      }
      __syncthreads();
    }
    tile_reduce_emit<T>(c, gt[0], gt[1], k, true, wc, wr, ad1, nullptr, cpre);
  }
}

template <typename T, int CX>
__global__ __launch_bounds__(kBlock) void k_interp_adj_march_n(const T* __restrict__ gfine, T* __restrict__ gcoarse,
                                                               T* __restrict__ gscaled, MarchArgs a, T scale,
                                                               AdamArgs<T> ad) {
  const int cny = a.cn[1], cnx = a.cn[2];
  const int fnz = a.fn[0], fny = a.fn[1], fnx = a.fn[2];
  const int64_t cplane = (int64_t)cny * cnx, fplane = (int64_t)fny * fnx;
  int z0, z1, jy, jx0;
  if (!march_decode<CX>(a, z0, z1, jy, jx0)) return;
  Adj6 ax[CX];
  column_taps<CX>(jx0, cnx, ax);
  const Adj6 ay = adj6(jy, cny);
  T pc[CX], pr[CX];
  {
    const int f1[1] = {2 * z0 - 1};
    T c1[1][CX], r1[1][CX];
    reduce_dispatch<T, CX, 1>(gfine, f1, fnz, fplane, fny, fnx, jy, jx0, ay, ax, c1, r1);
#pragma unroll
    for (int c = 0; c < CX; ++c) pc[c] = c1[0][c], pr[c] = r1[0][c];
  }
  for (int jz = z0; jz < z1; ++jz) {
    T c2[2][CX], r2[2][CX];
    const int f2[2] = {2 * jz, 2 * jz + 1};
    reduce_pair<T, CX>(gfine, f2, fnz, fplane, fny, fnx, jy, jx0, ay, ax, c2, r2);
    const int64_t ci = (int64_t)jz * cplane + (int64_t)jy * cnx + jx0;
#pragma unroll
    for (int c = 0; c < CX; ++c) {
      const T sc = c2[0][c] + T(0.5) * (pc[c] + c2[1][c]);
      T v = sc;
      if (ax[c].special || ay.special) {
        const T sr = r2[0][c] + T(0.5) * (pr[c] + r2[1][c]);
        v = T(2) * sc - sr;
      }
      pc[c] = c2[1][c], pr[c] = r2[1][c];
      emit_coarse<T>(gcoarse, gscaled, ci + c, v, scale, ad);
    }
  }
}

template <typename T, int CX, int NTAP>
__global__ __launch_bounds__(kBlock) void k_interp_adj_march_lead(const T* __restrict__ gfine,
                                                                  T* __restrict__ gcoarse, T* __restrict__ gscaled,
                                                                  MarchArgs a, T scale, AdamArgs<T> ad) {
  const int cnz = a.cn[0], cny = a.cn[1], cnx = a.cn[2];
  const int fnz = a.fn[0], fny = a.fn[1], fnx = a.fn[2];
  const int64_t cplane = (int64_t)cny * cnx, fplane = (int64_t)fny * fnx;
  const int64_t fvol = (int64_t)fnz * fplane;
  const int J0 = blockIdx.y;
  const bool node = a.lead_loc == kNode;
  int z0, z1, jy, jx0;
  if (!march_decode<CX>(a, z0, z1, jy, jx0)) return;
  if (ad.alpha_dev) ad.alpha_dev += (int64_t)J0 * ad.alpha_stride;
  Adj6 ax[CX];
  column_taps<CX>(jx0, cnx, ax);
  const Adj6 ay = adj6(jy, cny);
  int fv[3];
  T wv[3];
  if (node) {
#pragma unroll
    for (int t = 0; t < 3; ++t) {
      const int f = 2 * J0 - 1 + t;
      const bool ok = f >= 0 && f < a.lead_fn;
      fv[t] = ok ? f : 2 * J0;
      wv[t] = ok ? (t == 1 ? T(1) : T(0.5)) : T(0);
    }
  } else {
    fv[0] = fv[1] = fv[2] = J0;
    wv[0] = T(1);
    wv[1] = wv[2] = T(0);
  }
  T wc[NTAP][CX][6], wr[NTAP][CX][6];
#pragma unroll
  for (int t = 0; t < NTAP; ++t) {
    const T* gf = gfine + fv[t] * fvol;
    T c2[2][CX], r2[2][CX];
    const int fa[2] = {2 * z0 - 2, 2 * z0 - 1}, fb[2] = {2 * z0, 2 * z0 + 1};
    reduce_pair<T, CX>(gf, fa, fnz, fplane, fny, fnx, jy, jx0, ay, ax, c2, r2);
    put2<T, CX>(wc[t], wr[t], 0, c2, r2);
    reduce_pair<T, CX>(gf, fb, fnz, fplane, fny, fnx, jy, jx0, ay, ax, c2, r2);
    put2<T, CX>(wc[t], wr[t], 2, c2, r2);
  }
  for (int jz = z0; jz < z1; ++jz) {
    T v[CX];
#pragma unroll
    for (int c = 0; c < CX; ++c) v[c] = T(0);
#pragma unroll
    for (int t = 0; t < NTAP; ++t) {
      T c2[2][CX], r2[2][CX];
      const int fn2[2] = {2 * jz + 2, 2 * jz + 3};
      reduce_pair<T, CX>(gfine + fv[t] * fvol, fn2, fnz, fplane, fny, fnx, jy, jx0, ay, ax, c2, r2);
      put2<T, CX>(wc[t], wr[t], 4, c2, r2);
#pragma unroll
      for (int c = 0; c < CX; ++c)
        v[c] = v[c] + wv[t] * combine_z<T>(wc[t][c], wr[t][c], jz, cnz, fnz, ax[c].special || ay.special, 0, 0);
      slide<T, CX>(wc[t], wr[t]);
    }
    const int64_t ci = J0 * a.lead_cstride + (int64_t)jz * cplane + (int64_t)jy * cnx + jx0;
#pragma unroll
    for (int c = 0; c < CX; ++c) emit_coarse<T>(gcoarse, gscaled, ci + c, v[c], scale, ad);
  }
}

static bool march_setup(MarchArgs& m, const InterpArgs& a, int cx, int64_t target_units = 2 * kGridCap) {
  if ((a.loc[1] != kCell && a.loc[1] != kNode) || a.loc[2] != kCell || a.loc[3] != kCell) return false;
  if (a.loc[1] == kNode && a.cut_axis >= 0) return false;
  const bool lead = a.fn[0] != 1;
  if (a.loc[0] == kCell || (lead && (a.loc[1] != kCell || a.cut_axis >= 0 || a.fn[0] > 65535))) return false;
  m.lead_loc = lead ? a.loc[0] : 0;
  m.lead_cn = (int)a.cn[0];
  m.lead_fn = (int)a.fn[0];
  m.lead_cstride = a.coarse_ld ? a.coarse_ld : a.cn[1] * a.cn[2] * a.cn[3];
  if (a.coarse_ld && !lead) return false;
  for (int i = 0; i < 3; ++i) {
    if (a.fn[i + 1] >= (1 << 30)) return false;
    m.cn[i] = (int)a.cn[i + 1];
    m.fn[i] = (int)a.fn[i + 1];
  }
  if (m.cn[0] < 4) return false;
  m.nt = 0;
  m.cut_lo = a.cut_axis == 1 ? a.cut_lo : 0;
  m.cut_hi = a.cut_axis == 1 ? a.cut_hi : 0;
  if (a.cut_axis >= 0 && a.cut_axis != 1) return false;
  const int groups = (m.cn[2] + cx - 1) / cx;
  int tx = 1;
  while (tx < groups && tx < kBlock) tx *= 2;
  const int64_t xtiles = (groups + tx - 1) / tx;
  m.tx = tx;
  m.ty = kBlock / tx;
  const int64_t ytiles = (m.cn[1] + m.ty - 1) / m.ty;
  if ((int64_t)m.cn[0] * ytiles * xtiles >= ((int64_t)1 << 31)) return false;
  m.usched = make_unit_sched(m.cn[0], ytiles, xtiles, target_units);
  return true;
}

static inline bool aligned_to(const void* p, size_t bytes) { return (reinterpret_cast<uintptr_t>(p) % bytes) == 0; }

template <typename T>
static int march_cx(const InterpArgs& a, const void* f0, const void* f1) {
  const bool wide = sizeof(T) == 4 && a.cn[3] % 2 == 0 && a.cn[3] >= 4;
  if (wide && aligned_to(f0, 16) && (!f1 || aligned_to(f1, 16))) return 2;
  return aligned_to(f0, 2 * sizeof(T)) && (!f1 || aligned_to(f1, 2 * sizeof(T))) ? 1 : 0;
}

template <typename T, int CX>
static int add_launch(const T* coarse, const T* add, T* fine, const InterpArgs& a, T cscale, T ascale,
                      hipStream_t stream) {
  MarchArgs m;
  if (!march_setup(m, a, CX)) return 0;
  m.nt = (int64_t)m.lead_fn * m.fn[0] * m.fn[1] * m.fn[2] * (int64_t)sizeof(T) > kStreamBytes;
  const dim3 grid(unit_grid(m.usched), m.lead_fn);
  if (m.lead_fn != 1) {
// ... 224 lines not shown
  const char* e = getenv("ODIL_ADJ_ROWS");
  return !e || atoi(e) != 0;
}

template <typename T>
static bool adj_rows_plan(const MarchArgs& m, bool fine16, bool coarse8, RowsArgs& r) {
  if constexpr (sizeof(T) != 4) {
    return false;
  } else {
    const int fnx = m.fn[2];
    if (!adj_rows_enabled() || m.cut_lo || m.cut_hi || m.lead_loc == kNode) return false;
    if (fnx != 64 && fnx != 128 && fnx != 256) return false;
    for (int i = 0; i < 3; ++i)
      if (m.fn[i] != 2 * m.cn[i] || m.cn[i] < 4) return false;
    if (!fine16 || !coarse8) return false;
    if (m.lead_fn > 1 && (m.lead_cstride % 2) != 0) return false;
    for (int i = 0; i < 3; ++i) r.cn[i] = m.cn[i], r.fn[i] = m.fn[i];
    r.lxlog = fnx == 256 ? 6 : (fnx == 128 ? 5 : 4);
    const int planes_per_group = (kBlock / 64) * (64 >> r.lxlog);
    r.nzg = (m.cn[0] + planes_per_group - 1) / planes_per_group;
    const int64_t lead = m.lead_fn > 1 ? m.lead_fn : 1;
    r.yc = 32;
    while (r.yc > 8 && lead * r.nzg * ((m.cn[1] + r.yc - 1) / r.yc) < 4096) r.yc /= 2;
    r.nyc = (m.cn[1] + r.yc - 1) / r.yc;
    r.total = lead * r.nzg * r.nyc;
    r.per_xcd = (r.total + kNumXcd - 1) / kNumXcd;
    if (r.per_xcd * kNumXcd >= ((int64_t)1 << 31)) return false;
    r.fvol = (int64_t)m.fn[0] * m.fn[1] * m.fn[2];
    r.cvol = m.lead_cstride;
    return true;
  }
}

template <typename T>
static bool adj_rows_launch(const T* gfine, T* gcoarse, T* gscaled, const MarchArgs& m, T scale, hipStream_t stream,
                            const AdamArgs<T>& ad) {
  if constexpr (sizeof(T) != 4) {
    return false;
  } else {
    RowsArgs r;
    if (!adj_rows_plan<T>(m, aligned_to(gfine, 16), aligned_to(gcoarse, 8), r)) return false;
    hipLaunchKernelGGL(k_interp_adj_rows, dim3((unsigned)(r.per_xcd * kNumXcd)), dim3(kBlock), 0, stream, gfine, gcoarse,
                       gscaled, r, scale, ad);
    return true;
  }
}

template <typename T>
static void launch_adj_tile(dim3 grid, bool wide, hipStream_t stream, const T* gfine, T* gcoarse, T* gscaled,
                            const MarchArgs& m, T scale, const AdamArgs<T>& ad) {
  if constexpr (sizeof(T) == 4) {
    if (wide) {
      hipLaunchKernelGGL((k_interp_adj_tile<T, 2>), grid, dim3(kBlock), 0, stream, gfine, gcoarse, gscaled, m, scale, ad);
      return;
    }
  }
  hipLaunchKernelGGL((k_interp_adj_tile<T, 1>), grid, dim3(kBlock), 0, stream, gfine, gcoarse, gscaled, m, scale, ad);
}

static bool adj_tile_enabled() {
  const char* e = getenv("ODIL_ADJ_TILE");
  return !e || atoi(e) != 0;
}

static bool adj_small_level(const InterpArgs& a) { return a.cn[0] * a.cn[1] * a.cn[2] * a.cn[3] <= ((int64_t)1 << 22); }

static bool adj_tile_serves(const MarchArgs& m, const InterpArgs& a, int cx) {
  return cx == 1 && m.cn[1] >= 2 * kTileY && m.cn[2] >= 2 * kTileX && adj_tile_enabled() && !a.coarse_ld;
}

template <typename T>
int interp_adj_kind(const InterpArgs& a) {
  MarchArgs m;
  if (!march_setup(m, a, 1, adj_small_level(a) ? ODIL_ADJ_UNITS_SMALL : ODIL_ADJ_UNITS))
    return interp_fast_serves(a) ? kAdjFast : kAdjGeneric;
  if (m.lead_fn != 1 ? m.lead_loc == kNode : a.loc[1] == kNode) return kAdjNode;
  RowsArgs r;
  if (adj_rows_plan<T>(m, true, true, r)) return kAdjRows;
  return adj_tile_serves(m, a, 1) ? kAdjTile : kAdjMarch;
}
template int interp_adj_kind<double>(const InterpArgs&);
template int interp_adj_kind<float>(const InterpArgs&);

template <typename T, int CX>
static int adj_launch(const T* gfine, T* gcoarse, T* gscaled, const InterpArgs& a, T scale, hipStream_t stream,
                      const AdamArgs<T>& ad) {
  MarchArgs m;
  const bool small_level = adj_small_level(a);
  if (!march_setup(m, a, CX, small_level ? ODIL_ADJ_UNITS_SMALL : ODIL_ADJ_UNITS)) return 0;
  const dim3 grid(unit_grid(m.usched), m.lead_cn);
  const bool tile_ok = adj_tile_serves(m, a, CX);
  const bool tile_wide = sizeof(T) == 4 && m.cn[2] % 2 == 0 && m.cn[2] >= 4 * kTileX && aligned_to(gfine, 16);
  const int tile_cols = kTileX * (tile_wide ? 2 : 1);
  if (m.lead_fn != 1) {
    if (m.lead_loc == kNode)
      hipLaunchKernelGGL((k_interp_adj_march_lead<T, CX, 3>), grid, dim3(kBlock), 0, stream, gfine, gcoarse, gscaled,
                         m, scale, ad);
    else if (adj_rows_launch<T>(gfine, gcoarse, gscaled, m, scale, stream, ad)) {
    } else if (tile_ok) {
      const int64_t ytiles = (m.cn[1] + kTileY - 1) / kTileY, xtiles = (m.cn[2] + tile_cols - 1) / tile_cols;
      m.tx = kTileX;
      m.ty = kTileY;
      const int64_t per_volume = kGridCap / m.lead_cn > 2 * ytiles * xtiles ? kGridCap / m.lead_cn : 2 * ytiles * xtiles;
      m.usched = make_unit_sched(m.cn[0], ytiles, xtiles, per_volume);
      launch_adj_tile<T>(dim3(unit_grid(m.usched), m.lead_cn), tile_wide, stream, gfine, gcoarse, gscaled, m, scale, ad);
    } else
      hipLaunchKernelGGL((k_interp_adj_march_lead<T, CX, 1>), grid, dim3(kBlock), 0, stream, gfine, gcoarse, gscaled,
                         m, scale, ad);
  } else if (a.loc[1] == kNode)
    hipLaunchKernelGGL((k_interp_adj_march_n<T, CX>), grid, dim3(kBlock), 0, stream, gfine, gcoarse, gscaled, m, scale,
                       ad);
  else if (adj_rows_launch<T>(gfine, gcoarse, gscaled, m, scale, stream, ad)) {
  } else if (tile_ok) {
    const int64_t ytiles = (m.cn[1] + kTileY - 1) / kTileY, xtiles = (m.cn[2] + tile_cols - 1) / tile_cols;
    m.tx = kTileX;
    m.ty = kTileY;
    m.usched = make_unit_sched(m.cn[0], ytiles, xtiles, small_level ? ODIL_ADJ_UNITS_SMALL : ODIL_TILE_UNITS);
    launch_adj_tile<T>(dim3(unit_grid(m.usched)), tile_wide, stream, gfine, gcoarse, gscaled, m, scale, ad);
  } else
    hipLaunchKernelGGL((k_interp_adj_march<T, CX>), grid, dim3(kBlock), 0, stream, gfine, gcoarse, gscaled, m, scale,
                       ad);
  const int e = check_launch("k_interp_adj_march");
  return e ? e : 1;
}

template <typename T>
int poisson_adjoint_transpose(const T* fu, T* g0, T* g1, const int64_t* fshape, const T* h2, T scale,
                              const AdamArgs<T>& ad0, const AdamArgs<T>& ad1, int cut_lo, int cut_hi,
                              hipStream_t stream) {
  if (!fu || !g1 || !fshape || !h2) {
    set_error("poisson_adjoint_transpose: null pointer (fu, g1, shape, h2)");
    return ODIL_E_INVAL;
  }
  MarchArgs m;
  for (int i = 0; i < 3; ++i) {
    if (fshape[i] < 4 || fshape[i] % 2 || fshape[i] >= (1 << 30)) {
      set_error("poisson_adjoint_transpose: extent %lld on axis %d must be even, >= 4", (long long)fshape[i], i);
      return ODIL_E_INVAL;
    }
    m.fn[i] = (int)fshape[i];
    m.cn[i] = (int)(fshape[i] / 2);
  }
  const void* ptrs[] = {fu, g0, g1, ad0.x, ad0.m, ad0.v};
  for (const void* q : ptrs)
    if (q && !aligned_to(q, 2 * sizeof(T))) {
      set_error("poisson_adjoint_transpose: arrays must be aligned to %d bytes", (int)(2 * sizeof(T)));
      return ODIL_E_INVAL;
    }
  m.tx = kTileX, m.ty = kTileY;
  m.cut_lo = cut_lo, m.cut_hi = cut_hi;
  m.nt = 0;
  m.lead_loc = 0, m.lead_cn = 1, m.lead_fn = 1;
  const int64_t ytiles = (m.cn[1] + kTileY - 1) / kTileY, xtiles = (m.cn[2] + kTileX - 1) / kTileX;
  if ((int64_t)m.cn[0] * ytiles * xtiles >= ((int64_t)1 << 31)) {
    set_error("poisson_adjoint_transpose: grid too large for one launch");
    return ODIL_E_INVAL;
  }
  m.usched = make_unit_sched(m.cn[0], ytiles, xtiles, 2 * kGridCap);
  T h[3] = {h2[0], h2[1], h2[2]};
  const H2<T> hh = make_h2<T>(h);
  const bool mul = hh.mul_ok[0] && hh.mul_ok[1] && hh.mul_ok[2];
  const dim3 grid(unit_grid(m.usched));
#define ODIL_LAUNCH_ADJ_TILE(MUL, G0)                                                                             \
  hipLaunchKernelGGL((k_poisson_adjoint_tile<T, MUL, G0>), grid, dim3(kBlock), 0, stream, fu, g0, g1, m, hh, scale, \
                     ad0, ad1.x, ad1.m, ad1.v)
  if (mul && !g0) ODIL_LAUNCH_ADJ_TILE(true, false);
  else if (mul) ODIL_LAUNCH_ADJ_TILE(true, true);
  else if (!g0) ODIL_LAUNCH_ADJ_TILE(false, false);
  else ODIL_LAUNCH_ADJ_TILE(false, true);
#undef ODIL_LAUNCH_ADJ_TILE
  return check_launch("k_poisson_adjoint_tile");
}

template int poisson_adjoint_transpose<double>(const double*, double*, double*, const int64_t*, const double*, double,
                                               const AdamArgs<double>&, const AdamArgs<double>&, int, int, hipStream_t);
template int poisson_adjoint_transpose<float>(const float*, float*, float*, const int64_t*, const float*, float,
                                              const AdamArgs<float>&, const AdamArgs<float>&, int, int, hipStream_t);

template <typename T>
int interp_add_march(const T* coarse, const T* add, T* fine, const InterpArgs& a, T cscale, T ascale,
                     hipStream_t stream) {
  const int cx = march_cx<T>(a, fine, add);
  if constexpr (sizeof(T) == 4) {
    if (cx == 2) return add_launch<T, 2>(coarse, add, fine, a, cscale, ascale, stream);
  }
  return cx ? add_launch<T, 1>(coarse, add, fine, a, cscale, ascale, stream) : 0;
}

template <typename T>
int interp_adj_march(const T* gfine, T* gcoarse, T* gscaled, const InterpArgs& a, T scale, hipStream_t stream,
                     const AdamArgs<T>& ad) {
  return march_cx<T>(a, gfine, nullptr) ? adj_launch<T, 1>(gfine, gcoarse, gscaled, a, scale, stream, ad) : 0;
}

template int interp_add_march<double>(const double*, const double*, double*, const InterpArgs&, double, double,
                                      hipStream_t);
template int interp_add_march<float>(const float*, const float*, float*, const InterpArgs&, float, float, hipStream_t);
template int interp_adj_march<double>(const double*, double*, double*, const InterpArgs&, double, hipStream_t,
                                      const AdamArgs<double>&);
template int interp_adj_march<float>(const float*, float*, float*, const InterpArgs&, float, hipStream_t,
                                     const AdamArgs<float>&);

}

using namespace odil;

extern "C" {
int odil_poisson_adjoint_transpose_adam_f64(const double* fu, double* g0, double* g1, const int64_t* fshape,
                                            const double* h2, double scale, double* x0, double* m0, double* v0,
                                            double* x1, double* m1, double* v1, double alpha, double one_minus_b1,
                                            double one_minus_b2, double eps, const double* alpha_dev, int cut_lo,
                                            int cut_hi, void* stream) {
  const AdamArgs<double> a0{x0, m0, v0, alpha, one_minus_b1, one_minus_b2, eps, alpha_dev};
  const AdamArgs<double> a1{x1, m1, v1, alpha, one_minus_b1, one_minus_b2, eps, alpha_dev};
  return poisson_adjoint_transpose<double>(fu, g0, g1, fshape, h2, scale, a0, a1, cut_lo, cut_hi, (hipStream_t)stream);
}
int odil_poisson_adjoint_transpose_adam_f32(const float* fu, float* g0, float* g1, const int64_t* fshape,
                                            const float* h2, float scale, float* x0, float* m0, float* v0, float* x1,
                                            float* m1, float* v1, float alpha, float one_minus_b1, float one_minus_b2,
                                            float eps, const float* alpha_dev, int cut_lo, int cut_hi, void* stream) {
  const AdamArgs<float> a0{x0, m0, v0, alpha, one_minus_b1, one_minus_b2, eps, alpha_dev};
  const AdamArgs<float> a1{x1, m1, v1, alpha, one_minus_b1, one_minus_b2, eps, alpha_dev};
  return poisson_adjoint_transpose<float>(fu, g0, g1, fshape, h2, scale, a0, a1, cut_lo, cut_hi, (hipStream_t)stream);
}
}
```

### odil_amd/csrc/poisson_synth_tile.hip

```cpp
#include "poisson_synth.h"

namespace odil {

constexpr int kTileY = 8, kTileX = 32;
static_assert(kTileY * kTileX == kBlock, "one thread per coarse column");
constexpr int kCoarseRows = kTileY + 2, kCoarsePitch = kTileX + 2;
constexpr int kCoarseCells = kCoarseRows * kCoarsePitch;
constexpr int kStageRounds = (kCoarseCells + kBlock - 1) / kBlock;
constexpr int kFineRows = 2 * kTileY + 2, kFinePitch = 2 * kTileX + 4;
constexpr int kRingPairs = 2 * kTileX + 2 * kTileY, kHaloTasks = 2 * kRingPairs;
static_assert(kHaloTasks <= kBlock, "one ring pair per thread");

struct SynthTileArgs {
  int cn[3];
  UnitSched usched;
  int64_t loss_z0, loss_z1;
};

__device__ __forceinline__ int coarse_slot(int q) { return (q + 1) % 3; }

template <typename T>
__device__ inline T synth_val_staged(const T* c0, const T* c1, int sz, int sy, int sx, int base) {
  T s = T(0);
#pragma unroll
  for (int rz = 0; rz < 2; ++rz) {
    const T* c = rz ? c1 : c0;
#pragma unroll
    for (int ry = 0; ry < 2; ++ry)
#pragma unroll
      for (int rx = 0; rx < 2; ++rx) {
        const int w = (sz == rz ? 1 : 3) * (sy == ry ? 1 : 3) * (sx == rx ? 1 : 3);
        s = s + T(w) * c[base + ry * kCoarsePitch + rx];
      }
  }
  return s * (T(1) / T(64));
}

template <typename T>
struct StepLoads {
  PackN<T, 2> wC[2], wD[2], rB[2], rC[2];
  T ring[2];
};

template <typename T>
__device__ __forceinline__ void residual_tile_walk(const T* __restrict__ coarse, const T* __restrict__ w0,
                                                   const T* __restrict__ rhs, T* __restrict__ fu,
                                                   const SynthTileArgs& a, const H2<T>& h,
                                                   double* __restrict__ column_sums) {
  __shared__ T cs[3][kCoarseCells];
  __shared__ T fs[2][kFineRows * kFinePitch];
  const int cnz = a.cn[0], cny = a.cn[1], cnx = a.cn[2];
  const int FZ = 2 * cnz, FY = 2 * cny, FX = 2 * cnx;
  const int64_t cplane = (int64_t)cny * cnx, fplane = (int64_t)FY * FX;
  int zc, yt, xt;
  if (!unit_decode(a.usched, zc, yt, xt)) return;
  const int tid = threadIdx.x, lx = tid % kTileX, ly = tid / kTileX;
  const int jy0 = yt * kTileY, jx0 = xt * kTileX;
  const int jy = jy0 + ly, jx = jx0 + lx;
  const bool valid = jy < cny && jx < cnx;
  const int z0 = zc * a.usched.ZC;
  const int z1 = z0 + a.usched.ZC < cnz ? z0 + a.usched.ZC : cnz;
  const int fy0 = 2 * jy, fx0 = 2 * jx;
  const int64_t row0 = (int64_t)(2 * (jy < cny ? jy : cny - 1)) * FX + 2 * (jx < cnx ? jx : cnx - 1), row1 = row0 + FX;

  int64_t scl[kStageRounds], srf[kStageRounds];
  bool sout[kStageRounds];
#pragma unroll
  for (int k = 0; k < kStageRounds; ++k) {
    const int p = tid + k * kBlock < kCoarseCells ? tid + k * kBlock : kCoarseCells - 1;
    const int qy = jy0 - 1 + p / kCoarsePitch, qx = jx0 - 1 + p % kCoarsePitch;
    const int ycl = qy < 0 ? 0 : (qy >= cny ? cny - 1 : qy), yrf = qy < 0 ? 1 : (qy >= cny ? cny - 2 : qy);
    const int xcl = qx < 0 ? 0 : (qx >= cnx ? cnx - 1 : qx), xrf = qx < 0 ? 1 : (qx >= cnx ? cnx - 2 : qx);
    scl[k] = (int64_t)ycl * cnx + xcl;
    srf[k] = (int64_t)yrf * cnx + xrf;
    sout[k] = qy < 0 || qy >= cny || qx < 0 || qx >= cnx;
  }
  auto stage_load = [&](int q, T (&cl)[kStageRounds], T (&rf)[kStageRounds]) {
    const int zcl = q < 0 ? 0 : (q >= cnz ? cnz - 1 : q);
    const int zrf = q < 0 ? 1 : (q >= cnz ? cnz - 2 : q);
    const T* ccl = coarse + zcl * cplane;
    const T* crf = coarse + zrf * cplane;
#pragma unroll
    for (int k = 0; k < kStageRounds; ++k) {
      cl[k] = ccl[scl[k]];
      rf[k] = crf[srf[k]];
    }
  };
  auto stage_store = [&](int q, const T (&cl)[kStageRounds], const T (&rf)[kStageRounds]) {
    const bool oz = q < 0 || q >= cnz;
    const T cscale = T(1);
    T* plane = cs[coarse_slot(q)];
#pragma unroll
    for (int k = 0; k < kStageRounds; ++k) {
      const T val = cscale * cl[k];
      const T ghost = T(2) * val - cscale * rf[k];
      if (tid + k * kBlock < kCoarseCells) plane[tid + k * kBlock] = (oz || sout[k]) ? ghost : val;
    }
  };

  const int hz = tid / kRingPairs, hs = tid % kRingPairs;
  int hy, hx, hdy, hdx;
  if (hs < kTileX)
    hy = -1, hx = 2 * hs, hdy = 0, hdx = 1;
  else if (hs < 2 * kTileX)
    hy = 2 * kTileY, hx = 2 * (hs - kTileX), hdy = 0, hdx = 1;
  else if (hs < 2 * kTileX + kTileY)
    hy = 2 * (hs - 2 * kTileX), hx = -1, hdy = 1, hdx = 0;
  else
    hy = 2 * (hs - 2 * kTileX - kTileY), hx = 2 * kTileX, hdy = 1, hdx = 0;
  int64_t hoff[2];
  int hfine[2];
  int hbase[2], hsy[2], hsx[2];
#pragma unroll
  for (int c = 0; c < 2; ++c) {
    const int y = hy + c * hdy, x = hx + c * hdx;
    int gy = 2 * jy0 + y, gx = 2 * jx0 + x;
    gy = gy < 0 ? 0 : (gy >= FY ? FY - 1 : gy);
    gx = gx < 0 ? 0 : (gx >= FX ? FX - 1 : gx);
    hoff[c] = (int64_t)gy * FX + gx;
    hfine[c] = (1 + y) * kFinePitch + 2 + x;
    hsy[c] = y & 1, hsx[c] = x & 1;
    hbase[c] = ((y >> 1) + hsy[c]) * kCoarsePitch + (x >> 1) + hsx[c];
  }

  auto step_loads = [&](int jz, StepLoads<T>& s) {
    const int fzB = 2 * jz, fzC = 2 * jz + 1, fzD = 2 * jz + 2;
    const int64_t pB = (int64_t)fzB * fplane, pC = (int64_t)fzC * fplane;
    const int64_t pD = (int64_t)(fzD >= FZ ? FZ - 1 : fzD) * fplane;
    s.wC[0] = stream_ld<T, 2>(w0 + pC + row0, false);
    s.wC[1] = stream_ld<T, 2>(w0 + pC + row1, false);
    s.wD[0] = stream_ld<T, 2>(w0 + pD + row0, false);
    s.wD[1] = stream_ld<T, 2>(w0 + pD + row1, false);
    s.rB[0] = stream_ld<T, 2>(rhs + pB + row0, true);
    s.rB[1] = stream_ld<T, 2>(rhs + pB + row1, true);
    s.rC[0] = stream_ld<T, 2>(rhs + pC + row0, true);
    s.rC[1] = stream_ld<T, 2>(rhs + pC + row1, true);
    if (tid < kHaloTasks) {
      const T* wp = w0 + (hz ? pC : pB);
      s.ring[0] = wp[hoff[0]];
      s.ring[1] = wp[hoff[1]];
    }
  };

  StepLoads<T> cur;
  cur.ring[0] = cur.ring[1] = T(0);
  PackN<T, 2> wa[2], wb[2];
  {
    T cl[3][kStageRounds], rf[3][kStageRounds];
#pragma unroll
    for (int d = 0; d < 3; ++d) stage_load(z0 - 1 + d, cl[d], rf[d]);
    const int64_t pa = (int64_t)(z0 == 0 ? 0 : 2 * z0 - 1) * fplane, pb = (int64_t)(2 * z0) * fplane;
    wa[0] = stream_ld<T, 2>(w0 + pa + row0, false);
    wa[1] = stream_ld<T, 2>(w0 + pa + row1, false);
    wb[0] = stream_ld<T, 2>(w0 + pb + row0, false);
    wb[1] = stream_ld<T, 2>(w0 + pb + row1, false);
#pragma unroll
    for (int d = 0; d < 3; ++d) stage_store(z0 - 1 + d, cl[d], rf[d]);
  }
  __syncthreads();
  T v[3][3][3];
  auto read_window = [&](int q, T (&w)[3][3]) {
    const T* plane = cs[coarse_slot(q)];
#pragma unroll
    for (int dy = 0; dy < 3; ++dy)
#pragma unroll
      for (int dx = 0; dx < 3; ++dx) w[dy][dx] = plane[(ly + dy) * kCoarsePitch + lx + dx];
  };
  read_window(z0 - 1, v[0]);
  read_window(z0, v[1]);
  T uA[2][2], uB[2][2];
  synth_own<T, -1>(v, wa, uA);
  synth_own<T, 0>(v, wb, uB);

  double local = 0.0;
  const int own = (1 + 2 * ly) * kFinePitch + 2 + 2 * lx;
  for (int jz = z0; jz < z1; ++jz) {
    const int fzB = 2 * jz, fzC = 2 * jz + 1;
    const bool more = jz + 1 < z1;
    T ncl[kStageRounds], nrf[kStageRounds];
    step_loads(jz, cur);
    if (more) stage_load(jz + 2, ncl, nrf);
    read_window(jz + 1, v[2]);
    T uC[2][2], uD[2][2];
    synth_own<T, 1>(v, cur.wC, uC);
    synth_own<T, 2>(v, cur.wD, uD);
#pragma unroll
    for (int iy = 0; iy < 2; ++iy)
#pragma unroll
      for (int ix = 0; ix < 2; ++ix) {
        fs[0][own + iy * kFinePitch + ix] = uB[iy][ix];
        fs[1][own + iy * kFinePitch + ix] = uC[iy][ix];
      }
    if (tid < kHaloTasks) {
      const T* c0 = cs[coarse_slot(jz - 1 + hz)];
      const T* c1 = cs[coarse_slot(jz + hz)];
#pragma unroll
      for (int c = 0; c < 2; ++c)
        fs[hz][hfine[c]] = T(1) * cur.ring[c] + synth_val_staged<T>(c0, c1, hz, hsy[c], hsx[c], hbase[c]);
    }
    __syncthreads();
    T fB[2][2], fC[2][2];
#pragma unroll
    for (int ez = 0; ez < 2; ++ez) {
      const T* f = fs[ez] + own;
      T ylo[2], yhi[2], xlo[2], xhi[2];
#pragma unroll
      for (int i = 0; i < 2; ++i) {
        ylo[i] = f[-kFinePitch + i];
        yhi[i] = f[2 * kFinePitch + i];
        xlo[i] = f[i * kFinePitch - 1];
        xhi[i] = f[i * kFinePitch + 2];
      }
      if (ez == 0)
        residual_cells<T>(uB, uA, uC, ylo, yhi, xlo, xhi, cur.rB, fzB, fy0, fx0, FZ, FY, FX, h, fB);
      else
        residual_cells<T>(uC, uB, uD, ylo, yhi, xlo, xhi, cur.rC, fzC, fy0, fx0, FZ, FY, FX, h, fC);
    }
    if (fu && valid) {
      const int64_t pB = (int64_t)fzB * fplane, pC = (int64_t)fzC * fplane;
#pragma unroll
      for (int iy = 0; iy < 2; ++iy) {
        PackN<T, 2> o;
        o.e[0] = fB[iy][0], o.e[1] = fB[iy][1];
        stream_st<T, 2>(fu + pB + row0 + iy * FX, o, true);
        o.e[0] = fC[iy][0], o.e[1] = fC[iy][1];
        stream_st<T, 2>(fu + pC + row0 + iy * FX, o, true);
      }
    }
    const bool inB = fzB >= a.loss_z0 && fzB < a.loss_z1, inC = fzC >= a.loss_z0 && fzC < a.loss_z1;
#pragma unroll
    for (int iy = 0; iy < 2; ++iy)
#pragma unroll
      for (int ix = 0; ix < 2; ++ix) {
        if (inB) local += (double)(fB[iy][ix] * fB[iy][ix]);
        if (inC) local += (double)(fC[iy][ix] * fC[iy][ix]);
      }
    if (more) stage_store(jz + 2, ncl, nrf);
    __syncthreads();
#pragma unroll
    for (int iy = 0; iy < 2; ++iy)
#pragma unroll
      for (int ix = 0; ix < 2; ++ix) {
        uA[iy][ix] = uC[iy][ix];
        uB[iy][ix] = uD[iy][ix];
      }
#pragma unroll
    for (int dy = 0; dy < 3; ++dy)
#pragma unroll
      for (int dx = 0; dx < 3; ++dx) {
        v[0][dy][dx] = v[1][dy][dx];
        v[1][dy][dx] = v[2][dy][dx];
      }
  }
  if (valid) column_sums[((int64_t)zc * cny + jy) * cnx + jx] = local;
}

template <typename T>
__global__ __launch_bounds__(kBlock) void k_poisson_residual_tile(const T* __restrict__ coarse,
                                                                  const T* __restrict__ w0,
                                                                  const T* __restrict__ rhs, T* __restrict__ fu,
                                                                  SynthTileArgs a, H2<T> h,
                                                                  double* __restrict__ column_sums) {
  residual_tile_walk<T>(coarse, w0, rhs, fu, a, h, column_sums);
}

template <typename T>
__global__ __launch_bounds__(kBlock) void k_poisson_residual_tile_batch(const T* __restrict__ coarse,
                                                                        const T* __restrict__ w0,
                                                                        const T* __restrict__ rhs, T* __restrict__ fu,
                                                                        BatchStrides st, SynthTileArgs a, H2<T> h,
                                                                        double* __restrict__ column_sums) {
  const int64_t b = blockIdx.y;
  residual_tile_walk<T>(coarse + b * st.s[3], w0 + b * st.s[0], rhs + b * st.s[1], fu + b * st.s[2], a, h,
                        column_sums + b * st.s[4]);
}

__device__ __forceinline__ void synth_loss_replay(const double* __restrict__ column_sums, const MarchArgs& a,
                                                  double* __restrict__ partials) {
  const int cny = a.cn[1], cnx = a.cn[2];
  double local = 0.0;
  int zc, yt, xt;
  const bool have = unit_decode(a.usched, zc, yt, xt);
  const int lx = threadIdx.x % a.tx, ly = threadIdx.x / a.tx;
  const int jy = yt * a.ty + ly, jx = xt * a.tx + lx;
  if (have && jy < cny && jx < cnx) local = column_sums[((int64_t)zc * cny + jy) * cnx + jx];
  const double total = block_sum(local);
  if (threadIdx.x == 0) partials[blockIdx.x] = total;
}

__global__ __launch_bounds__(kBlock) void k_synth_loss_replay(const double* __restrict__ column_sums, MarchArgs a,
                                                              double* __restrict__ partials) {
  synth_loss_replay(column_sums, a, partials);
}

__global__ __launch_bounds__(kBlock) void k_synth_loss_replay_batch(const double* __restrict__ column_sums,
                                                                    int64_t sums_stride, MarchArgs a,
                                                                    double* __restrict__ partials,
                                                                    int64_t partials_stride) {
  const int64_t b = blockIdx.y;
  synth_loss_replay(column_sums + b * sums_stride, a, partials + b * partials_stride);
}

static size_t column_sums_bytes(const SynthArgs& sa) {
  return (size_t)sa.m.usched.ZCH * sa.m.cn[1] * sa.m.cn[2] * sizeof(double);
}

template <typename T>
static int poisson_residual_synth(const T* coarse, const T* w0, const T* rhs, T* fu, const int64_t* cshape,
                                  const T* h2, int64_t z0, int64_t z1, double denom, double* partials,
                                  double* column_sums, size_t column_sums_size, T* loss, void* stream) {
  if (!coarse || !w0 || !rhs || !partials || !column_sums || !loss) {
    set_error("poisson_residual_synth: null pointer");
    return ODIL_E_INVAL;
  }
  SynthArgs sa;
  if (int e = synth_geometry<T>(w0, rhs, fu, cshape, sa)) return e;
  const MarchArgs& m = sa.m;
  const int grid = unit_grid(m.usched);
  if (grid > kMaxPartials) {
    set_error("poisson_residual_synth: %d workgroups exceed the reduction workspace", grid);
    return ODIL_E_INVAL;
  }
  if (column_sums_size < column_sums_bytes(sa)) {
    set_error("poisson_residual_synth: column sums need %lld bytes, %lld given", (long long)column_sums_bytes(sa),
              (long long)column_sums_size);
    return ODIL_E_INVAL;
  }
  SynthTileArgs ta;
  for (int i = 0; i < 3; ++i) ta.cn[i] = m.cn[i];
  const int64_t ytiles = (m.cn[1] + kTileY - 1) / kTileY, xtiles = (m.cn[2] + kTileX - 1) / kTileX;
  if ((int64_t)m.usched.ZCH * (ytiles + kNumXcd) * xtiles >= ((int64_t)1 << 31)) {
    set_error("poisson_residual_synth: grid too large for one launch");
    return ODIL_E_INVAL;
  }
  ta.usched = make_unit_sched_chunked(m.cn[0], ytiles, xtiles, m.usched.ZC);
  ta.loss_z0 = z0;
  ta.loss_z1 = z1 < 0 ? m.fn[0] : z1;
  T hh[3] = {h2[0], h2[1], h2[2]};
  hipLaunchKernelGGL((k_poisson_residual_tile<T>), dim3(unit_grid(ta.usched)), dim3(kBlock), 0, (hipStream_t)stream,
                     coarse, w0, rhs, fu, ta, make_h2<T>(hh), column_sums);
  if (int e = check_launch("k_poisson_residual_tile")) return e;
  hipLaunchKernelGGL(k_synth_loss_replay, dim3(grid), dim3(kBlock), 0, (hipStream_t)stream, column_sums, m, partials);
  if (int e = check_launch("k_synth_loss_replay")) return e;
  const double size = denom > 0.0 ? denom : (double)m.fn[0] * m.fn[1] * m.fn[2];
  return launch_final_reduce<T>(partials, grid, 0, 1, size, loss, (hipStream_t)stream);
}

template <typename T>
static int poisson_residual_synth_batch(const T* coarse, const T* w0, const T* rhs, T* fu, int nbatch, int64_t w0_stride,
                                        int64_t rhs_stride, int64_t fu_stride, const int64_t* cshape, int ndim,
                                        const T* h2, double* partials, int64_t partials_stride, int64_t partials_len,
                                        double* column_sums, size_t column_sums_size, T* loss, void* stream) {
  static const char* what = "poisson_residual_synth_batch";
  if (ndim != 3) {
    set_error("%s: ndim %d (this ensemble runs 3-D members)", what, ndim);
    return ODIL_E_INVAL;
  }
  if (!coarse || !w0 || !rhs || !fu || !cshape || !h2 || !partials || !column_sums || !loss) {
    set_error("%s: null pointer", what);
    return ODIL_E_INVAL;
  }
  if (nbatch < 1 || nbatch > 65535) {
    set_error("%s: %d members (1 ... 65535, one grid row each)", what, nbatch);
    return ODIL_E_INVAL;
  }
  SynthArgs sa;
  if (int e = synth_geometry<T>(w0, rhs, fu, cshape, sa)) return e;
  const MarchArgs& m = sa.m;
  const int64_t cells = (int64_t)m.fn[0] * m.fn[1] * m.fn[2];
  const int64_t strides[3] = {w0_stride, rhs_stride, fu_stride};
  for (int k = 0; k < 3; ++k) {
    if (strides[k] < cells) {
      set_error("%s: member stride %lld is smaller than a member (%lld cells)", what, (long long)strides[k],
                (long long)cells);
      return ODIL_E_INVAL;
    }
    if ((strides[k] * (int64_t)sizeof(T)) % 16 != 0) {
      set_error("%s: member stride %lld is not a multiple of 16 bytes", what, (long long)strides[k]);
      return ODIL_E_INVAL;
    }
  }
  const int grid = unit_grid(m.usched);
  if (grid > kMaxPartials) {
    set_error("%s: %d workgroups exceed the reduction workspace", what, grid);
    return ODIL_E_INVAL;
  }
  if (partials_stride < grid || partials_stride >= ((int64_t)1 << 31)) {
    set_error("%s: partials workspace too small: rows of %lld doubles, a member needs %d", what,
              (long long)partials_stride, grid);
    return ODIL_E_INVAL;
  }
  if (partials_len < (int64_t)(nbatch - 1) * partials_stride + grid) {
    set_error("%s: partials workspace too small: %lld doubles are fewer than %d rows of %lld", what,
              (long long)partials_len, nbatch, (long long)partials_stride);
    return ODIL_E_INVAL;
  }
  const size_t per_member = column_sums_bytes(sa);
  if (column_sums_size / (size_t)nbatch < per_member) {
    set_error("%s: column sums need %lld bytes per member, %lld given for %d members", what, (long long)per_member,
              (long long)column_sums_size, nbatch);
    return ODIL_E_INVAL;
  }
  SynthTileArgs ta;
  for (int i = 0; i < 3; ++i) ta.cn[i] = m.cn[i];
  const int64_t ytiles = (m.cn[1] + kTileY - 1) / kTileY, xtiles = (m.cn[2] + kTileX - 1) / kTileX;
  if ((int64_t)m.usched.ZCH * (ytiles + kNumXcd) * xtiles >= ((int64_t)1 << 31)) {
    set_error("%s: grid too large for one launch", what);
// ... 71 lines not shown
```

### odil_amd/optimizer.py

```python

import math
import os
from argparse import Namespace

import numpy as np
import torch

from . import ops


class Optimizer:

    def __init__(self, name=None, displayname=None, dtype=None):
        self.name, self.displayname = name, displayname or name
        self.dtype, self.pinfo, self.evals = dtype, None, 0

    def run(self, x0, loss_grad, epochs, callback=None, epoch_start=0, **kwargs):
        return x0, Namespace(evals=0, epochs=0)


class EarlyStopError(Exception):
    def __init__(self, msg, optinfo):
        super().__init__(msg)
        self.optinfo = optinfo


def pack_like(arrays, dtype=None):
    sizes = [int(a.numel()) for a in arrays]
    dtype = dtype or arrays[0].dtype
    flat = torch.empty(sum(sizes), dtype=dtype, device=arrays[0].device)
    views = [t.view(a.shape) for t, a in zip(flat.split(sizes), arrays)]
    return flat, views


def flat_base(arrays):
    if not arrays:
        return None
    a0 = arrays[0]
    ptr = a0.data_ptr()
    esize = a0.element_size()
    storage = a0.untyped_storage()
    total = 0
    for a in arrays:
        if not a.is_contiguous() or a.dtype != a0.dtype or a.untyped_storage().data_ptr() != storage.data_ptr():
            return None
        if a.data_ptr() != ptr + total * esize:
            return None
        total += a.numel()
    offset = (ptr - storage.data_ptr()) // esize
    return torch.empty(0, dtype=a0.dtype, device=a0.device).set_(storage, offset, (total,), (1,))


def copy_into(flat, views, arrays):
    base = flat_base(arrays)
    if base is not None and base.dtype == flat.dtype:
        if base.data_ptr() != flat.data_ptr():
            flat.copy_(base)
        return
    for v, a in zip(views, arrays):
        v.copy_(a)


_graph_runtime_ready = False


def _graph_wanted(numel, loss_grad, epochs):
    mode = os.environ.get("ODIL_GRAPH", "auto")
    if mode in ("0", "1"):
        return mode == "1" and torch.cuda.is_available()
    safe = getattr(loss_grad, "graph_safe", None)
    long_enough = epochs >= 500 or (_graph_runtime_ready and epochs >= 20)
    return torch.cuda.is_available() and numel <= (1 << 22) and long_enough and safe is not None and safe()


class _EpochGraph:

    def __init__(self, step, step_sizes, dtype, device, loss_grad):
        self.step = step
        self.refresh = getattr(loss_grad, "refresh", None)
        self.begin, self.end = getattr(loss_grad, "graph_begin", None), getattr(loss_grad, "graph_end", None)
        self.nrows = len(step_sizes)
        self.table = torch.tensor(np.array(step_sizes, dtype=np.float64), dtype=dtype, device=device)
        self.index = torch.zeros(1, dtype=torch.int64, device=device)
        self.alpha = torch.zeros((1,) + tuple(self.table.shape[1:]), dtype=dtype, device=device)
        self.graph, self.pinfo = None, None

    def _body(self):
        torch.index_select(self.table, 0, self.index, out=self.alpha)
        pinfo = self.step(self.alpha)
        self.index.add_(1)
        return pinfo

    def capture(self):
        from .util import printlog

        try:
            graph = torch.cuda.CUDAGraph()
            if self.begin is not None:
                self.begin(self.nrows)
            with torch.cuda.graph(graph):
                pinfo = self._body()
            self.pinfo_type = type(pinfo) if isinstance(pinfo, dict) else None
            self.pinfo = {k: dict.__getitem__(pinfo, k) for k in dict.keys(pinfo)} if self.pinfo_type else pinfo
        except Exception as e:
            printlog("odil_amd: hipGraph capture of the Adam epoch failed ({}: {}); running eagerly".format(
                type(e).__name__, str(e).splitlines()[0] if str(e) else ""))
            torch.cuda.synchronize()
            self.index.zero_()
            self.close()
            return False
        self.graph = graph
        global _graph_runtime_ready
        _graph_runtime_ready = True
        return True

    def close(self):
        if self.end is not None:
            self.end()

    def replay(self):
        if self.refresh is not None:
            self.refresh()
        self.graph.replay()
        return self.pinfo_type(**self.pinfo) if self.pinfo_type else self.pinfo


def _adam_step_size(lr, beta_1, beta_2, t):
    return lr * np.sqrt(1 - beta_2**t) / (1 - beta_1**t)


def _whole_epochs_stop(callback, epoch, last):
    nxt = getattr(callback, "next_active", None) if callback is not None else (lambda e: last)
    return min(last, max(epoch, nxt(epoch - 1)) if nxt is not None else epoch, epoch + 4095)


class AdamNativeOptimizer(Optimizer):
    def __init__(self, dtype=None, mod=None, **kwargs):
        super().__init__(name="adamn", displayname="AdamNative", dtype=dtype)
        self.mod = mod

    def run(self, x0, loss_grad, epochs=None, callback=None, lr=1e-3, epoch_start=0, beta_1=0.9, beta_2=0.999,
            epsilon=1e-7, jit=True, moments=None, steps_done=0, **kwargs):
        tdtype = x0[0].dtype
        npdt = np.float64 if tdtype == torch.float64 else np.float32
        lr, beta_1, beta_2 = npdt(lr), npdt(beta_1), npdt(beta_2)
        xf, x = pack_like(x0)
        copy_into(xf, x, x0)
        mf = torch.zeros_like(xf)
        vf = torch.zeros_like(xf)
        mviews = [t.view(a.shape) for t, a in zip(mf.split([a.numel() for a in x]), x)]
        vviews = [t.view(a.shape) for t, a in zip(vf.split([a.numel() for a in x]), x)]
        if moments is not None:
            copy_into(mf, mviews, moments[0])
            copy_into(vf, vviews, moments[1])
        scratch = dict(gf=None, gviews=None)

        def step(alpha):
            fused = getattr(loss_grad, "fused_adam", None)
            done = 0
            if fused is not None:
                res = fused(x, mviews, vviews, alpha, 1 - beta_1, 1 - beta_2, epsilon)
                if res is not None:
                    loss, grads, pinfo, done = res
            if not done:
                loss, grads, pinfo = loss_grad(x)
            g = flat_base(grads)
            if g is None or g.dtype != tdtype or g.numel() != xf.numel():
                if scratch["gf"] is None:
                    scratch["gf"], scratch["gviews"] = pack_like(x)
                copy_into(scratch["gf"], scratch["gviews"], grads)
                g = scratch["gf"]
            n0 = sum(int(a.numel()) for a in x[:done])
            if n0 < xf.numel():
                ops.adam_step(xf[n0:], mf[n0:], vf[n0:], g[n0:], alpha, 1 - beta_1, 1 - beta_2, epsilon)
            return pinfo

        def step_size(epoch):
            return _adam_step_size(lr, beta_1, beta_2, npdt(epoch - epoch_start + steps_done))

        first, last = epoch_start + 1, epoch_start + epochs
        epoch = first
        small = getattr(loss_grad, "small_epochs", None)
        runner = None
        if small is not None and epochs > 0:
            table = torch.tensor(np.array([step_size(e) for e in range(first, last + 1)], dtype=np.float64), dtype=tdtype,
                                 device=xf.device)
            runner = small(x, mviews, vviews, table, 1 - beta_1, 1 - beta_2, epsilon)
        while runner is not None and epoch <= last:
            stop = _whole_epochs_stop(callback, epoch, last)
            pinfo = runner(epoch - first, stop - epoch + 1)
            self.evals += stop - epoch + 1
            epoch = stop + 1
            if callback is not None and stop > 0:
                captured = [a.data_ptr() for a in x]
                callback(x, stop, pinfo)
                if [a.data_ptr() for a in x] != captured:
                    runner = None
        graph = None
        if last - epoch + 1 > 4 and _graph_wanted(xf.numel(), loss_grad, epochs):
            while epoch < first + 2:
                self.evals += 1
                pinfo = step(step_size(epoch))
                if callback is not None:
                    callback(x, epoch, pinfo)
                epoch += 1
            graph = _EpochGraph(step, [step_size(e) for e in range(epoch, last + 1)], tdtype, xf.device, loss_grad)
            if not graph.capture():
                graph = None
        captured = [a.data_ptr() for a in x]
        while epoch <= last:
            self.evals += 1
            pinfo = graph.replay() if graph is not None else step(step_size(epoch))
            if epoch > 0 and callback is not None:
                callback(x, epoch, pinfo)
                if graph is not None and [a.data_ptr() for a in x] != captured:
                    graph.close()
                    graph = None
            epoch += 1
        if graph is not None:
            graph.close()
        optinfo = Namespace()
        optinfo.epochs = epochs
        optinfo.evals = self.evals
        optinfo.m, optinfo.v = mviews, vviews
        return x, optinfo


    def run_ensemble(self, ensemble, epochs, callback=None, lr=1e-3, lrs=None, epoch_start=0, beta_1=0.9, beta_2=0.999,
                     epsilon=1e-7, **kwargs):
        tdtype = ensemble.dtype
        npdt = np.float64 if tdtype == torch.float64 else np.float32
        beta_1, beta_2 = npdt(beta_1), npdt(beta_2)
        first, last = epoch_start + 1, epoch_start + epochs
        steps = lambda rate: [_adam_step_size(npdt(rate), beta_1, beta_2, npdt(e - epoch_start)) for e in range(first, last + 1)]
        if lrs is not None and len(lrs) != ensemble.nbatch:
            raise ValueError("{} step sizes for {} members".format(len(lrs), ensemble.nbatch))
        from .fused import BatchedLaunches

        if isinstance(ensemble, BatchedLaunches):
            return self._run_ensemble_launches(ensemble, epochs, callback, steps(lr) if lrs is None else [steps(r) for r in lrs],
                                               epoch_start, 1 - beta_1, 1 - beta_2, epsilon)
        table = np.array(steps(lr) if lrs is None else [steps(rate) for rate in lrs], dtype=np.float64)
        table = torch.tensor(table, dtype=tdtype, device=ensemble.device)
        losses = torch.empty((ensemble.nbatch, max(epochs, 0)), dtype=tdtype, device=ensemble.device)
        norms = torch.empty_like(losses)
        ensemble.m.zero_()
        ensemble.v.zero_()
        epoch = first
        while epoch <= last:
            stop = _whole_epochs_stop(callback, epoch, last)
            a, b = epoch - first, stop - first + 1
            ensemble.epochs(table[..., a:b], losses[:, a:b], norms[:, a:b], 1 - beta_1, 1 - beta_2, epsilon)
            self.evals += stop - epoch + 1
# ... 387 lines not shown
            nskip += 1
            continue
        push_pair(s_old, y_old, s_y, None)

    while True:
        vec.scale_into(d, g, -1.0 / theta)
        if col > 0:
            order = np.asarray(slots)
            if pending is not None:
                p1, p2 = pending
            else:
                sg_, yg_ = vec.history_products(len(slots), [g])
                p1, p2 = yg_[0], sg_[0]
            pending = None
            yg = np.asarray(p1)[order]
            sg = np.asarray(p2)[order] * theta
            rbar = np.triu(sy[:col, :col])
            amat = np.diag(np.diag(sy[:col, :col])) + yy[:col, :col] / theta
            q1 = -solve_triangular(rbar, sg, lower=False, check_finite=False)
            q2 = -solve_triangular(rbar, yg + amat @ q1, trans=1, lower=False, check_finite=False)
            cy = np.zeros(len(slots))
            cs = np.zeros(len(slots))
            cy[order] = -q1 / theta**2
            cs[order] = -q2 / theta
            vec.history_lincomb(d, len(slots), cs, cy)

        vec.probe_direction(d, g)
        vec.copy(t, x)
        vec.copy(r, g)
        fold = f
        stpmx = big
        launched = False
        if first:
            first = False
            dtd, gd = vec.read_probes()[:2]
            stp = min(1.0 / math.sqrt(dtd), stpmx)
        else:
            stp = 1.0
            evaluate(stp)
            launched = True
            dtd, gd, gd_new, gmax_new, f_new = vec.read_probes()
        gdold = gd
        ls_failed = False
        if gd >= 0.0:
            ls_failed = True
        else:
            search = _Dcsrch(stpmax=stpmx)
            stp, task = search.start(stp, f, gd)
            ifun = 0
            while task == "FG":
                ifun += 1
                nfev += 1
                iback = ifun - 1
                if iback >= maxls:
                    ls_failed = True
                    break
                if not launched:
                    evaluate(stp)
                    _, _, gd_new, gmax_new, f_new = vec.read_probes()
                launched = False
                f, gd, sbgnrm = f_new, gd_new, gmax_new
                stp, task = search.step(stp, f, gd)
                if nfev > maxfun:
                    break
            if task.startswith("ERROR"):
                ls_failed = True
        if ls_failed:
            vec.copy(x, t)
            vec.copy(g, r)
            f = fold
            if col == 0:
                return dict(task="ABNORMAL_TERMINATION_IN_LNSRCH", warnflag=2, nit=nit, funcalls=nfev, f=f)
            col, slots, theta = 0, [], 1.0
            pending = None
            continue

        nit += 1
        if callback is not None:
            callback(x)
        if nit >= maxiter:
            return dict(task="STOP: TOTAL NO. of ITERATIONS REACHED LIMIT", warnflag=1, nit=nit, funcalls=nfev, f=f)
        if nfev > maxfun:
            return dict(task="STOP: TOTAL NO. of f AND g EVALUATIONS EXCEEDS LIMIT", warnflag=1, nit=nit,
                        funcalls=nfev, f=f)
        if sbgnrm <= pgtol:
            return dict(task="CONVERGENCE: NORM_OF_PROJECTED_GRADIENT_<=_PGTOL", warnflag=0, nit=nit, funcalls=nfev, f=f)
        ddum = max(abs(fold), abs(f), 1.0)
        if (fold - f) <= epsmch * factr * ddum:
            return dict(task="CONVERGENCE: REL_REDUCTION_OF_F_<=_FACTR*EPSMCH", warnflag=0, nit=nit, funcalls=nfev, f=f)

        vec.sub_into(r, g, r)
        if stp == 1.0:
            dr = gd - gdold
            ddum = -gdold
        else:
            dr = (gd - gdold) * stp
            vec.scale_into(d, d, stp)
            ddum = -gdold * stp
        if dr <= epsmch * ddum:
            nskip += 1
            pending = None
            continue
        push_pair(d, r, dr, stp * stp * dtd if stp != 1.0 else dtd)


class LbfgsbOptimizer(Optimizer):
    def __init__(self, pgtol=1e-16, m=50, maxls=50, factr=0, dtype=None, mod=None, **kwargs):
        super().__init__(name="lbfgsb", displayname="L-BFGS-B", dtype=dtype)
        self.mod = mod
        self.pgtol, self.m, self.maxls, self.factr = pgtol, m, maxls, factr

    def run(self, x0, loss_grad, epochs=None, callback=None, epoch_start=0, **kwargs):
        self.epoch = epoch_start
        tdtype = x0[0].dtype
        device = x0[0].device
        xe, xviews = pack_like(x0)
        copy_into(xe, xviews, x0)
        n = xe.numel()
        x = xe if tdtype == torch.float64 else xe.to(torch.float64)
        gbuf = torch.zeros(n, dtype=torch.float64, device=device)
        gviews = [t.view(a.shape) for t, a in zip(gbuf.split([a.numel() for a in x0]), x0)]

        ev = dict(count=0, graph=None, out=None, raw=None, begun=False)
        want_graph = _graph_wanted(n, loss_grad, epochs or 0)
        refresh, begin, end = (getattr(loss_grad, k, None) for k in ("refresh", "graph_begin", "graph_end"))

        def close_graph():
            if ev["begun"] and end is not None:
                end()
            ev.update(graph=None, begun=False)

        def evaluate():
            if ev["graph"] is not None:
                try:
                    if refresh is not None:
                        refresh()
                except RuntimeError:
                    close_graph()
                    return loss_grad(xviews)
                ev["graph"].replay()
                loss, grads, raw = ev["out"]
                return loss, grads, (raw[0](**raw[1]) if raw[0] is not None else raw[1])
            ev["count"] += 1
            if want_graph and ev["count"] == 3:
                from .util import printlog

                try:
                    graph = torch.cuda.CUDAGraph()
                    if begin is not None:
                        begin(4 * (epochs or 0) + 64)
                        ev["begun"] = True
                    if refresh is not None:
                        refresh()
                    with torch.cuda.graph(graph):
                        loss, grads, pinfo = loss_grad(xviews)
                    kind = type(pinfo) if isinstance(pinfo, dict) else None
                    raw = {k: dict.__getitem__(pinfo, k) for k in dict.keys(pinfo)} if kind else pinfo
                    ev.update(graph=graph, out=(loss, grads, (kind, raw)))
                    global _graph_runtime_ready
                    _graph_runtime_ready = True
                    graph.replay()
                    return loss, grads, (kind(**raw) if kind else raw)
                except Exception as e:
                    printlog("odil_amd: hipGraph capture of the L-BFGS evaluation failed ({}: {}); running eagerly".format(
                        type(e).__name__, str(e).splitlines()[0] if str(e) else ""))
                    torch.cuda.synchronize()
                    close_graph()
            return loss_grad(xviews)

        def fg(xflat):
            self.evals += 1
            if xflat.data_ptr() != xe.data_ptr():
                xe.copy_(xflat)
            loss, grads, pinfo = evaluate()
            self.pinfo = pinfo
            base = flat_base(grads)
            if base is not None and base.dtype == torch.float64 and base.numel() == n:
                g = base
            else:
                for gv, gi in zip(gviews, grads):
                    gv.copy_(gi)
                g = gbuf
            return loss, g

        def callback_wrap(xflat):
            self.epoch += 1
            if callback:
                if xflat.data_ptr() != xe.data_ptr():
                    xe.copy_(xflat)
                callback(xviews, self.epoch, self.pinfo)

        vec = LbfgsVectors(n, self.m, device)
        try:
            res = lbfgsb_minimize(
                x, fg, vec, maxiter=epochs, m=self.m, maxls=self.maxls, pgtol=self.pgtol, factr=self.factr,
                callback=callback_wrap,
            )
        finally:
            close_graph()
        if x.data_ptr() != xe.data_ptr():
            xe.copy_(x)
        optinfo = Namespace()
        optinfo.warnflag = res["warnflag"]
        optinfo.task = res["task"]
        optinfo.evals = res["funcalls"]
        optinfo.epochs = res["nit"]
        if optinfo.warnflag not in [0, 1] or optinfo.epochs < epochs:
            raise EarlyStopError(
                ", ".join("{:}={:}".format(k, res.get(k, "")) for k in ["warnflag", "task", "funcalls", "nit"]),
                optinfo,
            )
        return xviews, optinfo


def make_optimizer(name, dtype=None, mod=None, **kwargs):
    if name == "lbfgsb":
        return LbfgsbOptimizer(dtype=dtype, mod=mod, **kwargs)
    elif name == "adam" or name == "adamn":
        return AdamNativeOptimizer(dtype=dtype, mod=mod, **kwargs)
    elif name == "gd":
        return GdOptimizer(dtype=dtype, mod=mod, **kwargs)
    elif name in ("lbfgs", "adam_tf"):
        raise ValueError("Optimizer '{}' is TensorFlow-specific; use 'lbfgsb' / 'adam'".format(name))
    raise ValueError("Unknown optimizer '{}'".format(name))
```

Measured before the change: 54.08 billion.

## Cost-balance adjoint tile units across XCDs and add specialised wall paths

Adds a cost-weighted partition of tile units across the 8 XCDs, so wall tiles that cost more are spread evenly instead of giving each XCD equal-count chunks. The adjoint tile kernel gains a Y-wall-only reduce path and per-axis specialised g0 plane kernels, so boundary tiles avoid the fully general code. Graph capture now disables Python GC, and optional unit-timing instrumentation plus a host helper that counts paths are added. The cost weights are hand-set constants, and the extra template paths raise code size.

```diff
diff --git a/include/odil_hip.h b/include/odil_hip.h
--- a/include/odil_hip.h
+++ b/include/odil_hip.h
@@ -292,6 +292,7 @@
                                      void* stream);
 
 int odil_interp_adj_kind(const int64_t* cshape, int ndim, const char* loc, int elem_size);
+int odil_tile_wall_paths(int64_t cny, int64_t cnx, int64_t* out);
 int odil_mg_volumes_levels_ok(const int64_t* shapes, int nlvl, int ndim, int nbatch, int elem_size);
 size_t odil_poisson_residual_synth_batch_workspace_bytes(const int64_t* cshape);
 int64_t odil_poisson_residual_synth_batch_partials(const int64_t* cshape);
diff --git a/odil_amd/_lib.py b/odil_amd/_lib.py
--- a/odil_amd/_lib.py
+++ b/odil_amd/_lib.py
@@ -98,7 +98,7 @@
     "odil_poisson_small_epochs_resident", "odil_poisson_small_epochs_partials", "odil_poisson_batch_partials",
     "odil_mg_batch_levels_ok", "odil_poisson_residual_synth_workspace_bytes",
     "odil_mg_volumes_levels_ok", "odil_interp_adj_kind", "odil_poisson_residual_synth_batch_workspace_bytes",
-    "odil_poisson_residual_synth_batch_partials",
+    "odil_poisson_residual_synth_batch_partials", "odil_tile_wall_paths",
 ] + [
     "odil_{}_{}".format(name, suffix) for name in _SIGNATURES for suffix in ("f64", "f32")
 ] + ["odil_{}_f64".format(name) for name in _SIGNATURES_F64]
@@ -142,6 +142,8 @@
     lib.odil_poisson_residual_synth_workspace_bytes.argtypes = [_I64P]
     lib.odil_interp_adj_kind.restype = c_int
     lib.odil_interp_adj_kind.argtypes = [_I64P, c_int, c_char_p, c_int]
+    lib.odil_tile_wall_paths.restype = c_int
+    lib.odil_tile_wall_paths.argtypes = [c_int64, c_int64, _I64P]
     lib.odil_mg_volumes_levels_ok.restype = c_int
     lib.odil_mg_volumes_levels_ok.argtypes = [_I64P, c_int, c_int, c_int, c_int]
     lib.odil_poisson_residual_synth_batch_workspace_bytes.restype = c_size_t
diff --git a/odil_amd/backend.py b/odil_amd/backend.py
--- a/odil_amd/backend.py
+++ b/odil_amd/backend.py
@@ -1,8 +1,23 @@
 
+import contextlib
+import gc
 from argparse import Namespace
 
 import numpy as np
 import torch
+
+
+@contextlib.contextmanager
+def graph_capture(graph):
+    gc.collect()
+    was_enabled = gc.isenabled()
+    gc.disable()
+    try:
+        with torch.cuda.graph(graph):
+            yield
+    finally:
+        if was_enabled:
+            gc.enable()
 
 _NP2T = {
     np.dtype("float32"): torch.float32,
diff --git a/odil_amd/core.py b/odil_amd/core.py
--- a/odil_amd/core.py
+++ b/odil_amd/core.py
@@ -8,7 +8,7 @@
 from torch.autograd.function import once_differentiable
 
 from . import ops
-from .backend import ModRocm, numpy_dtype, torch_dtype
+from .backend import ModRocm, graph_capture, numpy_dtype, torch_dtype
 
 
 def assert_equal(first, second, msg=""):
@@ -902,7 +902,7 @@
                     self._eval_loss_grad_generic(static_state)
             torch.cuda.current_stream().wait_stream(side)
             graph = torch.cuda.CUDAGraph()
-            with torch.cuda.graph(graph):
+            with graph_capture(graph):
                 out = self._eval_loss_grad_generic(static_state)
         finally:
             self.tracers = saved
diff --git a/odil_amd/csrc/common.h b/odil_amd/csrc/common.h
--- a/odil_amd/csrc/common.h
+++ b/odil_amd/csrc/common.h
@@ -6,6 +6,7 @@
 #include <string.h>
 
 #include "odil_hip.h"
+#include "unit_sched.h"
 
 namespace odil {
 
@@ -88,71 +89,50 @@
   return (int)(per_xcd * kNumXcd);
 }
 
-struct UnitSched {
-  int ZCH, Y, XS;
-  int ZC;
-  int axis;
-  int chunk;
-  int per_xcd;
-};
-
-inline UnitSched make_unit_sched_chunked(int64_t Z, int64_t Y, int64_t XS, int zc) {
-  UnitSched s;
-  s.ZC = zc;
-  s.ZCH = (int)((Z + zc - 1) / zc);
-  s.Y = (int)Y;
-  s.XS = (int)XS;
-  if (Y >= 4 * kNumXcd) {
-    s.axis = 1;
-    s.chunk = (int)((Y + kNumXcd - 1) / kNumXcd);
-    s.per_xcd = s.ZCH * s.chunk * s.XS;
-  } else if (s.ZCH >= kNumXcd) {
-    s.axis = 0;
-    s.chunk = 0;
-    s.per_xcd = (int)(((int64_t)s.ZCH * s.Y * s.XS + kNumXcd - 1) / kNumXcd);
-  } else {
-    s.axis = -1;
-    s.chunk = 0;
-    s.per_xcd = s.ZCH * s.Y * s.XS;
-  }
-  return s;
-}
-
-inline UnitSched make_unit_sched(int64_t Z, int64_t Y, int64_t XS, int64_t target_units = 2 * kGridCap) {
+static_assert(kSchedXcd == kNumXcd, "unit_sched.h splits over the XCDs of this chip");
+
+inline UnitSched make_unit_sched(int64_t Z, int64_t Y, int64_t XS, int64_t target_units = 2 * kGridCap,
+                                 UnitCost cost = UnitCost{0, 0, 0}) {
   int64_t zc = (Z * Y * XS) / target_units;
   if (zc < 1) zc = 1;
   if (zc > 64) zc = 64;
   if (zc > Z) zc = Z;
-  return make_unit_sched_chunked(Z, Y, XS, (int)zc);
-}
-
-inline int unit_grid(const UnitSched& s) { return s.axis < 0 ? s.per_xcd : s.per_xcd * kNumXcd; }
+  return make_unit_sched_chunked(Z, Y, XS, (int)zc, cost);
+}
 
 #ifdef __HIPCC__
 __device__ inline bool unit_decode(const UnitSched& s, int& zc, int& y, int& xs) {
-  if (s.axis < 0) {
-    const int i = blockIdx.x;
-    xs = i % s.XS;
-    const int r = i / s.XS;
-    y = r % s.Y;
-    zc = r / s.Y;
-    return true;
-  }
-  const int k = blockIdx.x % kNumXcd, i = blockIdx.x / kNumXcd;
-  xs = i % s.XS;
-  const int r = i / s.XS;
-  if (s.axis == 1) {
-    y = k * s.chunk + r % s.chunk;
-    zc = r / s.chunk;
-    return y < s.Y;
-  }
-  const int u = k * s.per_xcd + i;
-  xs = u % s.XS;
-  const int ru = u / s.XS;
-  y = ru % s.Y;
-  zc = ru / s.Y;
-  return zc < s.ZCH;
-}
+  return unit_decode_at(s, blockIdx.x, zc, y, xs);
+}
+#endif
+
+#if defined(ODIL_UNIT_TIMES) && defined(__HIPCC__)
+#define ODIL_UNIT_TIMES_ENTRY(name)                                                                          \
+  __device__ unsigned long long* g_unit_times_buf;                                                           \
+  __device__ long long g_unit_times_cap;                                                                     \
+  extern "C" int name(void* buf, long long records) {                                                        \
+    return hipMemcpyToSymbol(HIP_SYMBOL(g_unit_times_buf), &buf, sizeof(buf)) == hipSuccess &&               \
+                   hipMemcpyToSymbol(HIP_SYMBOL(g_unit_times_cap), &records, sizeof(records)) == hipSuccess  \
+               ? 0                                                                                           \
+               : ODIL_E_LAUNCH;                                                                              \
+  }
+#define ODIL_UNIT_TIMES_BEGIN(zc, y, xs)                                                                      \
+  if (threadIdx.x == 0 && g_unit_times_buf && (long long)blockIdx.x < g_unit_times_cap) {                     \
+    unsigned long long* rec_ = g_unit_times_buf + 4 * (long long)blockIdx.x;                                  \
+    rec_[0] = (unsigned long long)(zc) << 40 | (unsigned long long)(y) << 20 | (unsigned long long)(xs);      \
+    rec_[1] = wall_clock64();                                                                                 \
+  }
+#define ODIL_UNIT_TIMES_END()                                                                                 \
+  __syncthreads();                                                                                            \
+  if (threadIdx.x == 0 && g_unit_times_buf && (long long)blockIdx.x < g_unit_times_cap) {                     \
+    unsigned long long* rec_ = g_unit_times_buf + 4 * (long long)blockIdx.x;                                  \
+    rec_[2] = wall_clock64();                                                                                 \
+    rec_[3] = 1;                                                                                              \
+  }
+#else
+#define ODIL_UNIT_TIMES_ENTRY(name)
+#define ODIL_UNIT_TIMES_BEGIN(zc, y, xs)
+#define ODIL_UNIT_TIMES_END()
 #endif
 
 #ifdef __HIPCC__
diff --git a/odil_amd/csrc/mg_march.hip b/odil_amd/csrc/mg_march.hip
--- a/odil_amd/csrc/mg_march.hip
+++ b/odil_amd/csrc/mg_march.hip
@@ -649,6 +649,17 @@
 #ifndef ODIL_TILE_UNITS
 #define ODIL_TILE_UNITS (kGridCap / 2)
 #endif
+#ifndef ODIL_G0_AXES
+#define ODIL_G0_AXES 1
+#endif
+#ifndef ODIL_TILE_YWALL
+#define ODIL_TILE_YWALL 1
+#endif
+#ifndef ODIL_ADJ_COST_A
+#define ODIL_ADJ_COST_A 0.25f
+#define ODIL_ADJ_COST_B 0.18f
+#define ODIL_ADJ_COST_C 0.0f
+#endif
 constexpr int kTileY = ODIL_TILE_Y, kTileX = ODIL_TILE_X;
 constexpr int kTileR = 2 * kTileY + 4, kTileC = 2 * kTileX + 4;
 constexpr int kTilePacks = kTileR * (kTileC / 2);
@@ -657,17 +668,18 @@
 constexpr int kTileRS = kTileC / 2 + 2;
 constexpr int kTileLds = kTileR * kTileRS + 64;
 constexpr bool kTileStrips = (kBlock / 64) * (64 / kTileY) == kTileX;
-__device__ __forceinline__ void tile_column(int& lx, int& ly) {
+ODIL_HD inline void tile_column_of(int tid, int& lx, int& ly) {
   if constexpr (kTileStrips) {
     constexpr int W = 64 / kTileY;
-    const int wave = threadIdx.x >> 6, lane = threadIdx.x & 63;
+    const int wave = tid >> 6, lane = tid & 63;
     lx = wave * W + lane % W;
     ly = lane / W;
   } else {
-    lx = threadIdx.x % kTileX;
-    ly = threadIdx.x / kTileX;
-  }
-}
+    lx = tid % kTileX;
+    ly = tid / kTileX;
+  }
+}
+__device__ __forceinline__ void tile_column(int& lx, int& ly) { tile_column_of(threadIdx.x, lx, ly); }
 
 template <typename T, int CX = 1>
 struct TileVec {
@@ -687,6 +699,14 @@
     for (int i = 0; i < kTileLoads; ++i)
       pre[q][i] = *reinterpret_cast<const typename TileVec<T, CX>::type*>(gp + src[i]);
   }
+}
+
+enum TilePath : int { kPathInterior = 0, kPathX = 1, kPathY = 2, kPathGeneral = 3 };
+ODIL_HD inline int tile_lane_path(bool sx, bool sy, bool wave_sx, bool wave_sy, bool yw) {
+  if (!sx && !sy) return kPathInterior;
+  if (!wave_sy) return kPathX;
+  if (yw && !wave_sx) return kPathY;
+  return kPathGeneral;
 }
 
 template <typename T>
@@ -729,7 +749,7 @@
   }
 }
 
-template <typename T, int CX = 1, int RS = kTileRS>
+template <typename T, int CX = 1, int RS = kTileRS, bool YW = ODIL_TILE_YWALL != 0>
 __device__ __forceinline__ void tile_reduce_emit(const TileCtx<T>& c,
                                                  const typename TileVec<T, CX>::type* __restrict__ tile0,
                                                  const typename TileVec<T, CX>::type* __restrict__ tile1, int k,
@@ -742,8 +762,8 @@
   const int f2[2] = {2 * (c.z0 - 1 + k), 2 * (c.z0 - 1 + k) + 1};
   T c2[2][CX], r2[2][CX];
   const bool xy_special = c.sx || c.sy;
-  const bool wave_sy = __any(c.sy);
-  if (xy_special && !wave_sy) {
+  const int path = tile_lane_path(c.sx, c.sy, __any(c.sx), __any(c.sy), YW);
+  if (path == kPathX) {
     Adj6 ax[CX];
     if (wt) {
 #pragma unroll
@@ -785,7 +805,50 @@
 #pragma unroll
       for (int cc = 0; cc < CX; ++cc) c2[q][cc] = inside ? sc[cc] : T(0), r2[q][cc] = inside ? sr[cc] : T(0);
     }
-  } else if (xy_special) {
+  } else if (path == kPathY) {
+    float ywc[6], ywr[6];
+    if (wt) {
+#pragma unroll
+      for (int i = 0; i < 6; ++i) {
+        ywc[i] = wt[i * kBlock + threadIdx.x];
+        ywr[i] = wt[(6 + i) * kBlock + threadIdx.x];
+      }
+    } else {
+      const Adj6 ay = adj6(c.jy, c.cny);
+#pragma unroll
+      for (int i = 0; i < 6; ++i) ywc[i] = ay.wc[i], ywr[i] = ay.wr[i];
+    }
+#pragma unroll
+    for (int q = 0; q < 2; ++q) {
+      const P2* tq = q == 0 ? tile0 : tile1;
+      const bool inside = f2[q] >= 0 && f2[q] < c.fnz;
+      T sc[CX], sr[CX];
+#pragma unroll
+      for (int cc = 0; cc < CX; ++cc) sc[cc] = sr[cc] = T(0);
+#pragma unroll
+      for (int r = 0; r < 6; ++r) {
+        const T* rowv = reinterpret_cast<const T*>(tq + (2 * c.ly + r) * RS + lxl);
+        const P2 own = *reinterpret_cast<const P2*>(rowv + NV);
+        T val[NV + 2];
+        val[0] = rowv[NV - 1];
+#pragma unroll
+        for (int e = 0; e < NV; ++e) val[1 + e] = own[e];
+        val[NV + 1] = rowv[2 * NV];
+#pragma unroll
+        for (int cc = 0; cc < CX; ++cc) {
+          T xc = T(0);
+          xc = xc + T(0.25) * val[2 * cc];
+          xc = xc + T(0.75) * val[2 * cc + 1];
+          xc = xc + T(0.75) * val[2 * cc + 2];
+          xc = xc + T(0.25) * val[2 * cc + 3];
+          sc[cc] = sc[cc] + T(ywc[r]) * xc;
+          sr[cc] = sr[cc] + T(ywr[r]) * xc;
+        }
+      }
+#pragma unroll
+      for (int cc = 0; cc < CX; ++cc) c2[q][cc] = inside ? sc[cc] : T(0), r2[q][cc] = inside ? sr[cc] : T(0);
+    }
+  } else if (path == kPathGeneral) {
     Adj6 ax[CX], ay;
     if (wt) {
       tile_tables_load<CX>(wt, ay, ax);
@@ -983,6 +1046,46 @@
   return div_h2<T>(s, h, ax);
 }
 
+template <typename T, bool MUL, bool ZI, bool YI, bool XI>
+__device__ __forceinline__ void g0_plane(const typename TileVec<T>::type* __restrict__ pm,
+                                         const typename TileVec<T>::type* __restrict__ pc,
+                                         const typename TileVec<T>::type* __restrict__ pp,
+                                         typename TileVec<T>::type* __restrict__ gq, int fy0, int fx0, int fny, int fnx,
+                                         int zj, int zn, bool z_in, const H2<T>& h) {
+  typedef typename TileVec<T>::type P2;
+#pragma unroll 1
+  for (int i = 0; i < kG0Steps; ++i) {
+    const int w = threadIdx.x + i * kBlock;
+    const int r = w / kFuC, cc = w - r * kFuC;
+    if (r < kTileR && cc < kGC) {
+      const int y = fy0 - 2 + r, x = fx0 - 2 + 2 * cc;
+      const int at = w + kFuC + 1;
+      P2 g;
+      g[0] = T(0), g[1] = T(0);
+      if ((ZI || z_in) && (YI || (y >= 0 && y < fny)) && (XI || (x >= 0 && x < fnx))) {
+        const P2 fc = pc[at], fl = pc[at - 1], fr = pc[at + 1];
+        const P2 fym = pc[at - kFuC], fyp = pc[at + kFuC], fzm = pm[at], fzp = pp[at];
+#pragma unroll
+        for (int e = 0; e < 2; ++e) {
+          const T fb = fc[e];
+          const T xm = e == 0 ? fl[1] : fc[0], xp = e == 0 ? fc[1] : fr[0];
+          T acc = T(0);
+          if constexpr (ZI) acc = acc + lap_inner<T, MUL>(fb, fzm[e], fzp[e], h, 0);
+          else acc = acc + adj_axis<T>(fb, fzm[e], fzp[e], zj, zn, h, 0);
+          if constexpr (YI) acc = acc + lap_inner<T, MUL>(fb, fym[e], fyp[e], h, 1);
+          else acc = acc + adj_axis<T>(fb, fym[e], fyp[e], y, fny, h, 1);
+          if constexpr (XI) acc = acc + lap_inner<T, MUL>(fb, xm, xp, h, 2);
+          else acc = acc + adj_axis<T>(fb, xm, xp, x + e, fnx, h, 2);
+          g[e] = acc;
+        }
+      }
+      gq[r * kTileRS + cc] = g;
+    }
+  }
+}
+
+ODIL_UNIT_TIMES_ENTRY(odil_unit_times_adjoint)
+
 template <typename T, bool MUL, bool G0>
 __global__ __launch_bounds__(kBlock) void k_poisson_adjoint_tile(const T* __restrict__ fu, T* __restrict__ g0out_,
                                                                  T* __restrict__ gcoarse, MarchArgs a, H2<T> h,
@@ -997,6 +1100,7 @@
   const int cny = a.cn[1], fny = a.fn[1], fnx = a.fn[2];
   int zc, yt, xt;
   if (!unit_decode(a.usched, zc, yt, xt)) return;
+  ODIL_UNIT_TIMES_BEGIN(zc, yt, xt)
   if constexpr (MUL) h.mul_ok[0] = h.mul_ok[1] = h.mul_ok[2] = 1;
   if (ad0.alpha_dev) ad0.alpha = *ad0.alpha_dev;
   ad0.alpha_dev = nullptr;
@@ -1016,7 +1120,7 @@
   c.sx = c.owner && (c.jx < 2 || c.jx >= c.cnx - 2);
   c.sy = c.owner && (c.jy < 2 || c.jy >= cny - 2);
   const int fy0 = 2 * yt * kTileY, fx0 = 2 * xt * kTileX;
-  const bool tile_inner = fy0 >= 4 && fy0 + 2 * kTileY + 4 <= fny && fx0 >= 4 && fx0 + 2 * kTileX + 4 <= fnx;
+  const bool y_inner = fy0 >= 4 && fy0 + 2 * kTileY + 4 <= fny, x_inner = fx0 >= 4 && fx0 + 2 * kTileX + 4 <= fnx;
   int64_t src[kFuLoads];
 #pragma unroll
   for (int i = 0; i < kFuLoads; ++i) {
@@ -1103,59 +1207,20 @@
       P2* gq = gt[q];
       const int zj = z + (c.cut_lo ? 2 : 0), zn = c.fnz + (c.cut_lo ? 2 : 0) + (c.cut_hi ? 2 : 0);
       const bool z_in = z >= 0 && z < c.fnz;
-      if (tile_inner && z_in && zj >= 2 && zj < zn - 2) {
-#pragma unroll 1
-        for (int i = 0; i < kG0Steps; ++i) {
-          const int w = threadIdx.x + i * kBlock;
-          const int r = w / kFuC, cc = w - r * kFuC;
-          if (r < kTileR && cc < kGC) {
-            const int at = w + kFuC + 1;
-            const P2 fc = pc[at], fl = pc[at - 1], fr = pc[at + 1];
-            const P2 fym = pc[at - kFuC], fyp = pc[at + kFuC], fzm = pm[at], fzp = pp[at];
-            P2 g;
-#pragma unroll
-            for (int e = 0; e < 2; ++e) {
-              const T fb = fc[e];
-              T acc = T(0);
-              acc = acc + lap_inner<T, MUL>(fb, fzm[e], fzp[e], h, 0);
-              acc = acc + lap_inner<T, MUL>(fb, fym[e], fyp[e], h, 1);
-              acc = acc + lap_inner<T, MUL>(fb, e == 0 ? fl[1] : fc[0], e == 0 ? fc[1] : fr[0], h, 2);
-              g[e] = acc;
-            }
-            gq[r * kTileRS + cc] = g;
-          }
-        }
-      } else {
-#pragma unroll 1
-        for (int i = 0; i < kG0Steps; ++i) {
-          const int w = threadIdx.x + i * kBlock;
-          const int r = w / kFuC, cc = w - r * kFuC;
-          if (r < kTileR && cc < kGC) {
-            const int y = fy0 - 2 + r, x = fx0 - 2 + 2 * cc;
-            const int at = w + kFuC + 1;
-            P2 g;
-            g[0] = T(0), g[1] = T(0);
-            if (z_in && y >= 0 && y < fny && x >= 0 && x < fnx) {
-              const P2 fc = pc[at], fl = pc[at - 1], fr = pc[at + 1];
-              const P2 fym = pc[at - kFuC], fyp = pc[at + kFuC], fzm = pm[at], fzp = pp[at];
-#pragma unroll
-              for (int e = 0; e < 2; ++e) {
-                const T fb = fc[e];
-                T acc = T(0);
-                acc = acc + adj_axis<T>(fb, fzm[e], fzp[e], zj, zn, h, 0);
-                acc = acc + adj_axis<T>(fb, fym[e], fyp[e], y, fny, h, 1);
-                acc = acc + adj_axis<T>(fb, e == 0 ? fl[1] : fc[0], e == 0 ? fc[1] : fr[0], x + e, fnx, h, 2);
-                g[e] = acc;
-              }
-            }
-            gq[r * kTileRS + cc] = g;
-          }
-        }
-      }
+      const bool z_inner = z_in && zj >= 2 && zj < zn - 2;
+      if (z_inner && y_inner && x_inner)
+        g0_plane<T, MUL, true, true, true>(pm, pc, pp, gq, fy0, fx0, fny, fnx, zj, zn, z_in, h);
+      else if (ODIL_G0_AXES && z_inner && y_inner)
+        g0_plane<T, MUL, true, true, false>(pm, pc, pp, gq, fy0, fx0, fny, fnx, zj, zn, z_in, h);
+      else if (ODIL_G0_AXES && z_inner && x_inner)
+        g0_plane<T, MUL, true, false, true>(pm, pc, pp, gq, fy0, fx0, fny, fnx, zj, zn, z_in, h);
+      else
+        g0_plane<T, MUL, false, false, false>(pm, pc, pp, gq, fy0, fx0, fny, fnx, zj, zn, z_in, h);
       __syncthreads();
     }
     tile_reduce_emit<T>(c, gt[0], gt[1], k, true, wc, wr, ad1, nullptr, cpre);
   }
+  ODIL_UNIT_TIMES_END()
 }
 
 template <typename T, int CX>
@@ -1686,11 +1751,12 @@
   m.nt = 0;
   m.lead_loc = 0, m.lead_cn = 1, m.lead_fn = 1;
   const int64_t ytiles = (m.cn[1] + kTileY - 1) / kTileY, xtiles = (m.cn[2] + kTileX - 1) / kTileX;
-  if ((int64_t)m.cn[0] * ytiles * xtiles >= ((int64_t)1 << 31)) {
+  if ((int64_t)m.cn[0] * (ytiles + kNumXcd) * xtiles >= ((int64_t)1 << 31)) {
     set_error("poisson_adjoint_transpose: grid too large for one launch");
     return ODIL_E_INVAL;
   }
-  m.usched = make_unit_sched(m.cn[0], ytiles, xtiles, 2 * kGridCap);
+  m.usched = make_unit_sched(m.cn[0], ytiles, xtiles, 2 * kGridCap,
+                             UnitCost{ODIL_ADJ_COST_A, ODIL_ADJ_COST_B, ODIL_ADJ_COST_C});
   T h[3] = {h2[0], h2[1], h2[2]};
   const H2<T> hh = make_h2<T>(h);
   const bool mul = hh.mul_ok[0] && hh.mul_ok[1] && hh.mul_ok[2];
@@ -1740,6 +1806,33 @@
 using namespace odil;
 
 extern "C" {
+int odil_tile_wall_paths(int64_t cny, int64_t cnx, int64_t* out) {
+  if (!out || cny < 2 || cnx < 2 || cny >= (1 << 30) || cnx >= (1 << 30)) {
+    set_error("odil_tile_wall_paths: bad arguments");
+    return ODIL_E_INVAL;
+  }
+  for (int p = 0; p < 4; ++p) out[p] = 0;
+  const int64_t ytiles = (cny + kTileY - 1) / kTileY, xtiles = (cnx + kTileX - 1) / kTileX;
+  for (int64_t yt = 0; yt < ytiles; ++yt)
+    for (int64_t xt = 0; xt < xtiles; ++xt)
+      for (int wave = 0; wave < kBlock / 64; ++wave) {
+        bool sx[64], sy[64], wave_sx = false, wave_sy = false, seen[4] = {false, false, false, false};
+        for (int lane = 0; lane < 64; ++lane) {
+          int lx, ly;
+          tile_column_of(wave * 64 + lane, lx, ly);
+          const int64_t jy = yt * kTileY + ly, jx = xt * kTileX + lx;
+          const bool owner = jy < cny && jx < cnx;
+          sx[lane] = owner && (jx < 2 || jx >= cnx - 2);
+          sy[lane] = owner && (jy < 2 || jy >= cny - 2);
+          wave_sx = wave_sx || sx[lane], wave_sy = wave_sy || sy[lane];
+        }
+        for (int lane = 0; lane < 64; ++lane)
+          seen[tile_lane_path(sx[lane], sy[lane], wave_sx, wave_sy, ODIL_TILE_YWALL != 0)] = true;
+        for (int p = 0; p < 4; ++p) out[p] += seen[p];
+      }
+  return 0;
+}
+
 int odil_poisson_adjoint_transpose_adam_f64(const double* fu, double* g0, double* g1, const int64_t* fshape,
                                             const double* h2, double scale, double* x0, double* m0, double* v0,
                                             double* x1, double* m1, double* v1, double alpha, double one_minus_b1,
diff --git a/odil_amd/csrc/poisson_synth_tile.hip b/odil_amd/csrc/poisson_synth_tile.hip
--- a/odil_amd/csrc/poisson_synth_tile.hip
+++ b/odil_amd/csrc/poisson_synth_tile.hip
@@ -41,6 +41,8 @@
   PackN<T, 2> wC[2], wD[2], rB[2], rC[2];
   T ring[2];
 };
+
+ODIL_UNIT_TIMES_ENTRY(odil_unit_times_residual)
 
 template <typename T>
 __device__ __forceinline__ void residual_tile_walk(const T* __restrict__ coarse, const T* __restrict__ w0,
@@ -54,6 +56,7 @@
   const int64_t cplane = (int64_t)cny * cnx, fplane = (int64_t)FY * FX;
   int zc, yt, xt;
   if (!unit_decode(a.usched, zc, yt, xt)) return;
+  ODIL_UNIT_TIMES_BEGIN(zc, yt, xt)
   const int tid = threadIdx.x, lx = tid % kTileX, ly = tid / kTileX;
   const int jy0 = yt * kTileY, jx0 = xt * kTileX;
   const int jy = jy0 + ly, jx = jx0 + lx;
@@ -253,6 +256,7 @@
       }
   }
   if (valid) column_sums[((int64_t)zc * cny + jy) * cnx + jx] = local;
+  ODIL_UNIT_TIMES_END()
 }
 
 template <typename T>
diff --git a/odil_amd/csrc/unit_sched.h b/odil_amd/csrc/unit_sched.h
--- /dev/null
+++ b/odil_amd/csrc/unit_sched.h
@@ -0,0 +1,109 @@
+#pragma once
+#include <stdint.h>
+
+#ifdef __HIPCC__
+#define ODIL_HD __host__ __device__
+#else
+#define ODIL_HD
+#endif
+
+namespace odil {
+
+constexpr int kSchedXcd = 8;
+
+struct UnitSched {
+  int ZCH, Y, XS;
+  int ZC;
+  int axis;
+  int chunk;
+  int per_xcd;
+  int stride;
+  int bnd[kSchedXcd + 1];
+};
+
+struct UnitCost {
+  float a, b, c;
+};
+
+inline double unit_cost(const UnitCost& w, int y, int xs, int Y, int XS) {
+  const bool xw = xs == 0 || xs == XS - 1, yw = y == 0 || y == Y - 1;
+  return 1.0 + (xw ? w.a : 0.0) + (yw ? w.b : 0.0) + (xw && yw ? w.c : 0.0);
+}
+
+inline UnitSched make_unit_sched_chunked(int64_t Z, int64_t Y, int64_t XS, int zc, UnitCost cost = UnitCost{0, 0, 0}) {
+  UnitSched s;
+  s.ZC = zc;
+  s.ZCH = (int)((Z + zc - 1) / zc);
+  s.Y = (int)Y;
+  s.XS = (int)XS;
+  s.stride = 0;
+  for (int k = 0; k <= kSchedXcd; ++k) s.bnd[k] = 0;
+  if (Y >= 4 * kSchedXcd) {
+    s.axis = 1;
+    s.chunk = (int)((Y + kSchedXcd - 1) / kSchedXcd);
+    if (cost.a == 0 && cost.b == 0 && cost.c == 0) {
+      for (int k = 0; k <= kSchedXcd; ++k) {
+        const int64_t y = (int64_t)k * s.chunk < Y ? (int64_t)k * s.chunk : Y;
+        s.bnd[k] = (int)(y * XS);
+      }
+    } else {
+      double total = 0;
+      for (int y = 0; y < s.Y; ++y)
+        for (int xs = 0; xs < s.XS; ++xs) total += unit_cost(cost, y, xs, s.Y, s.XS);
+      const int n = s.Y * s.XS;
+      double before = 0;
+      int t = 0;
+      for (int k = 1; k < kSchedXcd; ++k) {
+        const double target = total * k / kSchedXcd;
+        while (t < n) {
+          const double ct = unit_cost(cost, t / s.XS, t % s.XS, s.Y, s.XS);
+          if (before + 0.5 * ct > target) break;
+          before += ct;
+          ++t;
+        }
+        s.bnd[k] = t;
+      }
+      s.bnd[kSchedXcd] = n;
+    }
+    for (int k = 0; k < kSchedXcd; ++k)
+      if (s.bnd[k + 1] - s.bnd[k] > s.stride) s.stride = s.bnd[k + 1] - s.bnd[k];
+    s.per_xcd = s.ZCH * s.stride;
+  } else if (s.ZCH >= kSchedXcd) {
+    s.axis = 0;
+    s.chunk = 0;
+    s.per_xcd = (int)(((int64_t)s.ZCH * s.Y * s.XS + kSchedXcd - 1) / kSchedXcd);
+  } else {
+    s.axis = -1;
+    s.chunk = 0;
+    s.per_xcd = s.ZCH * s.Y * s.XS;
+  }
+  return s;
+}
+
+inline int unit_grid(const UnitSched& s) { return s.axis < 0 ? s.per_xcd : s.per_xcd * kSchedXcd; }
+
+ODIL_HD inline bool unit_decode_at(const UnitSched& s, int b, int& zc, int& y, int& xs) {
+  if (s.axis < 0) {
+    xs = b % s.XS;
+    const int r = b / s.XS;
+    y = r % s.Y;
+    zc = r / s.Y;
+    return true;
+  }
+  const int k = b % kSchedXcd, i = b / kSchedXcd;
+  if (s.axis == 1) {
+    const int tl = i % s.stride, t = s.bnd[k] + tl;
+    zc = i / s.stride;
+    y = t / s.XS;
+    xs = t - y * s.XS;
+    return t < s.bnd[k + 1];
+  }
+  const int u = k * s.per_xcd + i;
+  xs = u % s.XS;
+  const int ru = u / s.XS;
+  y = ru % s.Y;
+  zc = ru / s.Y;
+  return zc < s.ZCH;
+}
+
+}
diff --git a/odil_amd/optimizer.py b/odil_amd/optimizer.py
--- a/odil_amd/optimizer.py
+++ b/odil_amd/optimizer.py
@@ -7,6 +7,7 @@
 import torch
 
 from . import ops
+from .backend import graph_capture
 
 
 class Optimizer:
@@ -98,7 +99,7 @@
             graph = torch.cuda.CUDAGraph()
             if self.begin is not None:
                 self.begin(self.nrows)
-            with torch.cuda.graph(graph):
+            with graph_capture(graph):
                 pinfo = self._body()
             self.pinfo_type = type(pinfo) if isinstance(pinfo, dict) else None
             self.pinfo = {k: dict.__getitem__(pinfo, k) for k in dict.keys(pinfo)} if self.pinfo_type else pinfo
@@ -792,7 +793,7 @@
                         ev["begun"] = True
                     if refresh is not None:
                         refresh()
-                    with torch.cuda.graph(graph):
+                    with graph_capture(graph):
                         loss, grads, pinfo = loss_grad(xviews)
                     kind = type(pinfo) if isinstance(pinfo, dict) else None
                     raw = {k: dict.__getitem__(pinfo, k) for k in dict.keys(pinfo)} if kind else pinfo
```

After: 53.75 billion. No clear change (-0.6%).
